# otiliastr/coper

Measured on NVIDIA B200. Metric: train_rows_per_s, higher is better.
Workload: dtype fp16x3

## Files before the change

### coper_b200/_lib.py

```python
from __future__ import annotations

import ctypes as C
import os

_HERE = os.path.dirname(os.path.abspath(__file__))
LIB_PATH = os.path.join(_HERE, "libcoper_sm100.so")

PREC = {"fp32": 0, "bf16": 1, "tf32x3": 2, "fp16x3": 3}
CPG_BWD_REUSE_FWD, CPG_BWD_INPUT_GRADS_ONLY, CPG_BWD_WEIGHT_GRADS_ONLY, CPG_BWD_DCB_ACCUMULATE = 1, 2, 4, 8

vp, i32, i64, u64, f32, sz = C.c_void_p, C.c_int, C.c_int64, C.c_uint64, C.c_float, C.c_size_t

SIGNATURES = {
    "coper_version": (i32, []),
    "coper_status_string": (C.c_char_p, [i32]),
    "coper_last_cuda_error": (i32, []),
    "coper_launch_count": (C.c_longlong, []),
    "coper_device_is_sm100": (i32, []),
    "coper_set_pdl": (i32, [i32]),
    "coper_gather_rows": (i32, [vp, i64, i64, i32, vp, i32, vp, vp]),
    "coper_gather_rows2": (i32, [vp, i64, i64, i32, vp, i32, vp, vp, i64, i64, i32, vp, i32, vp, vp, vp, f32, f32, f32, vp]),
    "coper_conv_fwd": (i32, [vp, i32, i32, i32, vp, vp, i32, i32, i32, i32, vp, vp]),
    "coper_conv_bwd_slabs": (i32, [i32, i32, i32, i32, i32, i32, i32]),
    "coper_conv_bwd": (i32, [vp, vp, i32, i32, i32, vp, i32, i32, i32, i32, vp, vp, vp, vp]),
    "coper_conv_bwd_bn": (i32, [vp, vp, vp, i32, i32, i32, vp, i32, i32, i32, i32, vp, vp, vp, vp, vp, vp, i32, f32, vp, u64,
                                vp, vp, vp, vp, vp]),
    "coper_colstats_chunks": (i32, [i64]),
    "coper_colstats": (i32, [vp, i64, i32, vp, vp]),
    "coper_bn_finalize": (i32, [vp, i32, i64, i32, vp, vp, vp, vp, f32, f32, i32, i32, i32, vp, vp, vp, vp, vp]),
    "coper_bn_stats_finalize": (i32, [vp, i64, i32, vp, vp, vp, vp, vp, vp, f32, f32, i32, i32, vp, vp, vp, vp, vp]),
    "coper_bn_act_fwd": (i32, [vp, i64, i32, vp, vp, i32, f32, vp, u64, vp, vp]),
    "coper_bn_act_fwd_moving": (i32, [vp, i64, i32, vp, vp, vp, vp, f32, i32, vp, vp]),
    "coper_bn_act_bwd_stats": (i32, [vp, vp, i64, i32, vp, vp, vp, vp, i32, f32, vp, u64, vp, vp]),
    "coper_bn_act_bwd_stats_finalize": (i32, [vp, vp, i64, i32, vp, vp, vp, vp, i32, f32, vp, u64, vp, vp, i32, vp, vp, vp, vp,
                                              vp]),
    "coper_bn_act_bwd_finalize": (i32, [vp, i32, i64, i32, i32, vp, vp, vp, vp, vp]),
    "coper_bn_act_bwd_apply": (i32, [vp, vp, i64, i32, vp, vp, vp, vp, vp, vp, i32, f32, vp, u64, f32, u64, vp, vp]),
    "coper_dropout_mask": (i32, [i64, f32, vp, u64, vp, vp]),
    "coper_dropout_apply": (i32, [vp, i64, f32, vp, u64, vp]),
    "coper_cpg_fc_fwd_workspace_bytes": (sz, [i32, i32, i32, i32, i32]),
    "coper_cpg_fc_fwd": (i32, [vp, vp, vp, vp, vp, vp, i32, i32, i32, i32, i32, f32, vp, u64, vp, vp, sz, i32, vp]),
    "coper_cpg_fc_bwd_workspace_bytes": (sz, [i32, i32, i32, i32, i32]),
    "coper_cpg_fc_bwd": (i32, [vp, vp, vp, vp, vp, vp, vp, i32, i32, i32, i32, i32, vp, vp, vp, vp, vp, vp, sz, i32, i32,
                               vp]),
    "coper_sgemm": (i32, [i32, i32, i32, i32, i32, vp, i32, vp, i32, vp, i32, i32, vp]),
    "coper_score1n_workspace_bytes": (sz, [i32, i64, i32, i32]),
    "coper_score1n_fwd": (i32, [vp, vp, vp, i32, i64, i32, vp, i64, vp, sz, i32, vp]),
    "coper_prepared_bytes": (sz, [i64, i32, i32]),
    "coper_prepare_operand": (i32, [vp, i64, i32, i64, i32, vp, vp]),
    "coper_score1n_fwd_prepared": (i32, [vp, vp, vp, i32, i64, i32, vp, i64, i32, vp]),
    "coper_tc_gemm_workspace_bytes": (sz, [i32, i32, i32, i32]),
    "coper_tc_gemm": (i32, [i32, i32, i32, i32, i32, vp, i32, vp, i32, vp, i32, i32, vp, sz, vp]),
    "coper_score1n_bce_workspace_bytes": (sz, [i32, i64, i32, i32]),
    "coper_score1n_bce_G_bytes": (sz, [i32, i64, i32]),
    "coper_score1n_bce_fwd_bwd": (i32, [vp, vp, vp, vp, vp, i32, i64, i32, f32, f32, f32, vp, vp, i64, vp, vp, vp, vp,
                                        sz, i32, vp]),
    "coper_score1n_bce_fwd_bwd_norm": (i32, [vp, vp, vp, vp, vp, i32, i64, i32, f32, f32, f32, vp, vp, i64, vp, vp, vp, vp,
                                             vp, sz, i32, vp]),
    "coper_score1n_bce_dE": (i32, [vp, i32, i64, i32, f32, vp, vp, vp, vp, sz, i32, vp]),
    "coper_sample_labels": (i32, [vp, vp, i32, i64, i32, i32, vp, u64, vp, vp, vp]),
    "coper_score_sampled_workspace_bytes": (sz, [i32, i32]),
    "coper_score_sampled_bce_fwd_bwd": (i32, [vp, vp, vp, vp, vp, i32, i32, i64, i32, f32, f32, f32, vp, vp, vp, vp, vp,
                                              vp, vp, vp, vp, sz, vp]),
    "coper_score_sampled_sharded_workspace_bytes": (sz, [i32, i32]),
    "coper_score_sampled_bce_fwd_bwd_sharded": (i32, [vp, vp, vp, vp, vp, i32, i32, i64, i32, f32, f32, f32, vp, vp, vp,
                                                      vp, vp, vp, vp, vp, i64, i64, vp, sz, vp]),
    "coper_score_candidates": (i32, [vp, vp, vp, vp, i32, i32, i32, i64, i64, vp, vp]),
    "coper_candidate_rank": (i32, [vp, vp, vp, vp, vp, i32, i32, i32, i64, i64, vp, vp, i32, vp, vp, vp]),
    "coper_csr_to_bits": (i32, [vp, vp, i32, i64, i64, vp, vp]),
    "coper_dense_to_bits": (i32, [vp, i32, i64, vp, vp]),
    "coper_gold_scores": (i32, [vp, i64, i32, i64, vp, i64, vp, vp]),
    "coper_filtered_rank": (i32, [vp, i64, i32, i64, vp, i64, vp, vp, vp, vp, vp]),
    "coper_score1n_rank_workspace_bytes": (sz, [i32, i32, i32]),
    "coper_score1n_gold_prepared": (i32, [vp, vp, vp, i32, i64, i32, vp, i64, vp, vp, sz, i32, vp]),
    "coper_score1n_rank_prepared": (i32, [vp, vp, vp, i32, i64, i32, vp, vp, vp, vp, i32, vp]),
    "coper_score1n_topk_workspace_bytes": (sz, [i32, i64, i32, i32, i32]),
    "coper_score1n_topk_prepared": (i32, [vp, vp, vp, i32, i64, i32, vp, i64, i32, vp, vp, vp, sz, i32, vp]),
    "coper_topk_scores_workspace_bytes": (sz, [i32, i64, i32]),
    "coper_topk_scores": (i32, [vp, i64, i32, i64, vp, i64, i32, vp, vp, vp, sz, vp]),
    "coper_topk_merge": (i32, [vp, vp, i32, i32, i32, vp, vp, vp]),
    "coper_csr_to_bits_t": (i32, [vp, vp, i32, i64, i64, vp, vp]),
    "coper_dense_to_bits_t": (i32, [vp, i32, i64, i64, vp, vp]),
    "coper_bits_t_set": (i32, [vp, i32, i64, i64, vp, vp]),
    "coper_segscatter_workspace_bytes": (sz, [i32]),
    "coper_segscatter_add_sq": (i32, [vp, i32, vp, i32, vp, vp, i64, i64, vp]),
    "coper_segscatter_add_norm": (i32, [vp, i32, vp, i32, vp, vp, i64, i64, vp, vp]),
    "coper_segscatter_add_pair": (i32, [vp, i32, vp, i32, vp, vp, i64, i64, vp, vp, i32, vp, i32, vp, vp, i64, i64, vp]),
    "coper_segscatter_add": (i32, [vp, i32, vp, i32, vp, i64, i64, vp, sz, vp]),
    "coper_reduce_partials": (i32, [vp, i32, i64, f32, i32, vp, vp]),
    "coper_reduce_partials2": (i32, [vp, i64, vp, vp, i64, vp, i32, f32, i32, vp]),
    "coper_sumsq": (i32, [vp, i64, i32, vp, vp]),
    "coper_clip_scale": (i32, [vp, i32, f32, vp, vp]),
    "coper_step_state_advance": (i32, [vp, vp, f32, f32, f32, vp]),
    "coper_sumsq_combine": (i32, [vp, i32, vp, i32, vp, vp]),
    "coper_mt_sumsq": (i32, [vp, i32, vp, i32, vp, vp, vp, vp]),
    "coper_clip_scale_n": (i32, [vp, i32, f32, vp, vp]),
    "coper_mt_sumsq_clip": (i32, [vp, i32, vp, i32, vp, vp, vp, i32, vp, i32, vp, i32, f32, vp, vp]),
    "coper_mt_amsgrad": (i32, [vp, vp, i32, vp, f32, f32, f32, vp, i32, vp]),
    "coper_amsgrad_step": (i32, [vp, vp, vp, vp, vp, i64, vp, f32, f32, f32, vp, i32, vp]),
}
SUMSQ_BLOCKS = 256
TOPK_MAX = 128
MT_CHUNK = 16384

_lib = None
launch_count = 0


class CoperError(RuntimeError):
    pass


def load():
    global _lib
    if _lib is not None:
        return _lib
    if not os.path.exists(LIB_PATH):
        raise CoperError(
            "libcoper_sm100.so not found at %s — build it with `python -m coper_b200.build` "
            "(there is no CPU/PyTorch fallback for the CoPER hot path)" % LIB_PATH)
    lib = C.CDLL(LIB_PATH)
    for name, (res, args) in SIGNATURES.items():
        fn = getattr(lib, name)
        fn.restype = res
        fn.argtypes = args
    _lib = lib
    return lib


def check(rc, what=""):
    if rc != 0:
        lib = load()
        msg = lib.coper_status_string(rc).decode()
        raise CoperError("%s failed: %s (status %d, cudaError %d)" % (what, msg, rc, lib.coper_last_cuda_error()))


def ptr(t):
    return None if t is None else t.data_ptr()


def stream_ptr():
    import torch
    return torch.cuda.current_stream().cuda_stream


def call_plain(name, *args):
    check(getattr(load(), name)(*args), name)


def call(name, *args):
    global launch_count
    lib = load()
    launch_count += 1
    check(getattr(lib, name)(*args, stream_ptr()), name)
```

### coper_b200/csrc/common.cuh

```cuda
#pragma once
#include <cuda_runtime.h>
#include <stdint.h>
#include "../../include/coper.h"

namespace coper {

extern thread_local int g_last_cuda_error;
extern long long g_launch_count;

inline int check_launch() {
  ++g_launch_count;
  cudaError_t e = cudaPeekAtLastError();
  if (e != cudaSuccess) {
    g_last_cuda_error = (int)e;
    cudaGetLastError();
    return COPER_ERR_CUDA;
  }
  return COPER_OK;
}
inline int check_cuda(cudaError_t e) {
  if (e != cudaSuccess) {
    g_last_cuda_error = (int)e;
    return COPER_ERR_CUDA;
  }
  return COPER_OK;
}
#define COPER_CHECK_ARG(cond) \
  do {                        \
    if (!(cond)) return COPER_ERR_INVALID_ARG; \
  } while (0)

static inline cudaStream_t as_stream(coper_stream_t s) { return reinterpret_cast<cudaStream_t>(s); }

__device__ __forceinline__ void pdl_trigger() { asm volatile("griddepcontrol.launch_dependents;" ::: "memory"); }
__device__ __forceinline__ void pdl_wait() { asm volatile("griddepcontrol.wait;" ::: "memory"); }
__device__ __forceinline__ void pdl_enter() {
  pdl_trigger();
  pdl_wait();
}
bool pdl_enabled();
template <typename... KArgs, typename... Args>
inline void launch_pdl(void (*kernel)(KArgs...), dim3 grid, dim3 block, size_t smem, cudaStream_t st, Args&&... args) {
  cudaLaunchConfig_t cfg = {};
  cfg.gridDim = grid;
  cfg.blockDim = block;
  cfg.dynamicSmemBytes = smem;
  cfg.stream = st;
  cudaLaunchAttribute attr[1];
  attr[0].id = cudaLaunchAttributeProgrammaticStreamSerialization;
  attr[0].val.programmaticStreamSerializationAllowed = pdl_enabled() ? 1 : 0;
  cfg.attrs = attr;
  cfg.numAttrs = 1;
  cudaLaunchKernelEx(&cfg, kernel, static_cast<KArgs>(args)...);
}

__host__ __device__ __forceinline__ uint32_t hash32(uint64_t seed, uint64_t idx) {
  uint64_t z = seed + (idx + 1) * 0x9E3779B97F4A7C15ull;
  z = (z ^ (z >> 30)) * 0xBF58476D1CE4E5B9ull;
  z = (z ^ (z >> 27)) * 0x94D049BB133111EBull;
  z ^= (z >> 31);
  return (uint32_t)(z >> 32);
}
__host__ __device__ __forceinline__ uint32_t keep_threshold(float keep) {
  double t = (double)keep * 4294967296.0;
  if (t >= 4294967295.0) return 0xFFFFFFFFu;
  if (t <= 0.0) return 0u;
  return (uint32_t)t;
}
__device__ __forceinline__ float drop_factor(float keep, float inv_keep, uint32_t thr, uint64_t seed, uint64_t idx) {
  if (keep >= 1.0f) return 1.0f;
  return hash32(seed, idx) < thr ? inv_keep : 0.0f;
}

__device__ __forceinline__ float bn_bwd_dx(float dout, float post_factor, float xv, float ac, float bc, float mean,
                                           float invstd, float c1, float c2, int relu) {
  float g = __fmul_rn(dout, post_factor);
  if (relu && !(fmaf(ac, xv, bc) > 0.f)) g = 0.f;
  const float xhat = __fmul_rn(__fsub_rn(xv, mean), invstd);
  return __fmul_rn(ac, fmaf(-xhat, c2, __fsub_rn(g, c1)));
}

__device__ __forceinline__ float warp_sum(float v) {
#pragma unroll
  for (int o = 16; o > 0; o >>= 1) v += __shfl_xor_sync(0xffffffffu, v, o);
  return v;
}
__device__ __forceinline__ float warp_max(float v) {
#pragma unroll
  for (int o = 16; o > 0; o >>= 1) v = fmaxf(v, __shfl_xor_sync(0xffffffffu, v, o));
  return v;
}
__device__ __forceinline__ double warp_sum_d(double v) {
#pragma unroll
  for (int o = 16; o > 0; o >>= 1) v += __shfl_xor_sync(0xffffffffu, v, o);
  return v;
}
__device__ __forceinline__ int warp_sum_i(int v) {
#pragma unroll
  for (int o = 16; o > 0; o >>= 1) v += __shfl_xor_sync(0xffffffffu, v, o);
  return v;
}

template <typename T>
__device__ __forceinline__ T block_sum(T v, T* smem32) {
  int lane = threadIdx.x & 31, w = threadIdx.x >> 5;
#pragma unroll
  for (int o = 16; o > 0; o >>= 1) v += __shfl_xor_sync(0xffffffffu, v, o);
  if (lane == 0) smem32[w] = v;
  __syncthreads();
  T r = T(0);
  if (w == 0) {
    int nw = (blockDim.x + 31) >> 5;
    r = lane < nw ? smem32[lane] : T(0);
#pragma unroll
    for (int o = 16; o > 0; o >>= 1) r += __shfl_xor_sync(0xffffffffu, r, o);
  }
  __syncthreads();
  return r;
}

constexpr int kFp16x3TargetExp = 10;
__host__ __device__ __forceinline__ int fp16x3_exponent_of(float absmax) {
  if (!(absmax > 0.f) || !(absmax < 3.0e38f)) return 0;
  int ex;
  frexpf(absmax, &ex);
  int e = kFp16x3TargetExp - (ex - 1);
  return e < -100 ? -100 : (e > 100 ? 100 : e);
}

inline int sm_count() {
  static int cached[64] = {};
  int dev = 0;
  if (cudaGetDevice(&dev) != cudaSuccess || dev < 0 || dev >= 64) return 148;
  if (!cached[dev]) {
    int n = 0;
    if (cudaDeviceGetAttribute(&n, cudaDevAttrMultiProcessorCount, dev) != cudaSuccess || n <= 0) n = 148;
    cached[dev] = n;
  }
  return cached[dev];
}

int reduce_partials_and_sum(const float* in, int S, int64_t n, float scale, int accumulate, float* out,
                            const double* dsum_in, int dsum_n, double* dsum_out, cudaStream_t st);

static inline int ceil_div(int64_t a, int64_t b) { return (int)((a + b - 1) / b); }
static inline size_t align_up(size_t x, size_t a) { return (x + a - 1) / a * a; }

}
```

### coper_b200/csrc/umma.cuh

```cuda
#pragma once
#include <cuda.h>
#include <cuda_bf16.h>
#include "common.cuh"

namespace coper {
namespace umma {

__device__ __forceinline__ uint32_t smem_u32(const void* p) { return (uint32_t)__cvta_generic_to_shared(p); }

__device__ __forceinline__ bool elect_one() {
  uint32_t pred;
  asm volatile("{\n\t.reg .pred P;\n\telect.sync _|P, 0xffffffff;\n\tselp.u32 %0, 1, 0, P;\n\t}" : "=r"(pred));
  return pred != 0;
}
__device__ __forceinline__ int warp_idx_uniform() { return __shfl_sync(0xffffffffu, (int)(threadIdx.x >> 5), 0); }

__device__ __forceinline__ void mbar_init(uint64_t* bar, uint32_t count) {
  asm volatile("mbarrier.init.shared::cta.b64 [%0], %1;" ::"r"(smem_u32(bar)), "r"(count));
}
__device__ __forceinline__ void fence_barrier_init() { asm volatile("fence.mbarrier_init.release.cluster;" ::: "memory"); }
__device__ __forceinline__ void fence_proxy_async() { asm volatile("fence.proxy.async.shared::cta;" ::: "memory"); }
__device__ __forceinline__ void mbar_expect_tx(uint64_t* bar, uint32_t bytes) {
  asm volatile("mbarrier.arrive.expect_tx.shared::cta.b64 _, [%0], %1;" ::"r"(smem_u32(bar)), "r"(bytes) : "memory");
}
__device__ __forceinline__ void mbar_arrive(uint64_t* bar) {
  asm volatile("mbarrier.arrive.shared::cta.b64 _, [%0];" ::"r"(smem_u32(bar)) : "memory");
}
__device__ __forceinline__ void mbar_wait(uint64_t* bar, uint32_t parity) {
  uint32_t addr = smem_u32(bar);
  uint32_t done = 0;
  while (!done) {
    asm volatile(
        "{\n\t.reg .pred p;\n\t"
        "mbarrier.try_wait.parity.shared::cta.b64 p, [%1], %2;\n\t"
        "selp.u32 %0, 1, 0, p;\n\t}"
        : "=r"(done)
        : "r"(addr), "r"(parity)
        : "memory");
  }
}

__device__ __forceinline__ void tma_load_2d(void* dst_smem, const CUtensorMap* tmap, uint64_t* bar, int c0, int c1) {
  asm volatile(
      "cp.async.bulk.tensor.2d.shared::cluster.global.mbarrier::complete_tx::bytes [%0], [%1, {%3, %4}], [%2];"
      ::"r"(smem_u32(dst_smem)), "l"(reinterpret_cast<uint64_t>(tmap)), "r"(smem_u32(bar)), "r"(c0), "r"(c1)
      : "memory");
}
__device__ __forceinline__ void tma_store_2d(const CUtensorMap* tmap, const void* src_smem, int c0, int c1) {
  asm volatile("cp.async.bulk.tensor.2d.global.shared::cta.bulk_group [%0, {%2, %3}], [%1];"
               ::"l"(reinterpret_cast<uint64_t>(tmap)), "r"(smem_u32(src_smem)), "r"(c0), "r"(c1)
               : "memory");
}
__device__ __forceinline__ void tma_store_commit() { asm volatile("cp.async.bulk.commit_group;" ::: "memory"); }
__device__ __forceinline__ void tma_store_wait_read() { asm volatile("cp.async.bulk.wait_group.read 0;" ::: "memory"); }
__device__ __forceinline__ void tma_store_wait_all() { asm volatile("cp.async.bulk.wait_group 0;" ::: "memory"); }
__device__ __forceinline__ void mbar_wait_guarded(uint64_t* bar, uint32_t parity) {
  uint32_t addr = smem_u32(bar);
  uint32_t done = 0;
  long long t0 = 0;
  for (uint32_t spins = 0; !done; ++spins) {
    asm volatile(
        "{\n\t.reg .pred p;\n\t"
        "mbarrier.try_wait.parity.shared::cta.b64 p, [%1], %2;\n\t"
        "selp.u32 %0, 1, 0, p;\n\t}"
        : "=r"(done)
        : "r"(addr), "r"(parity)
        : "memory");
    if (!done && (spins & 1023u) == 1023u) {
      long long now = clock64();
      if (t0 == 0) t0 = now;
      else if (now - t0 > 4000000000ll) __trap();
    }
  }
}
__device__ __forceinline__ void tma_prefetch_l2_2d(const CUtensorMap* tmap, int c0, int c1) {
  asm volatile("cp.async.bulk.prefetch.tensor.2d.L2.global.tile [%0, {%1, %2}];"
               ::"l"(reinterpret_cast<uint64_t>(tmap)), "r"(c0), "r"(c1)
               : "memory");
}
__device__ __forceinline__ void tma_prefetch_desc(const CUtensorMap* tmap) {
  asm volatile("prefetch.tensormap [%0];" ::"l"(reinterpret_cast<uint64_t>(tmap)) : "memory");
}

__device__ __forceinline__ void tmem_alloc(uint32_t* smem_dst, uint32_t ncols) {
  asm volatile("tcgen05.alloc.cta_group::1.sync.aligned.shared::cta.b32 [%0], %1;" ::"r"(smem_u32(smem_dst)), "r"(ncols)
               : "memory");
}
__device__ __forceinline__ void tmem_relinquish() {
  asm volatile("tcgen05.relinquish_alloc_permit.cta_group::1.sync.aligned;" ::: "memory");
}
__device__ __forceinline__ void tmem_dealloc(uint32_t taddr, uint32_t ncols) {
  asm volatile("tcgen05.dealloc.cta_group::1.sync.aligned.b32 %0, %1;" ::"r"(taddr), "r"(ncols) : "memory");
}
__device__ __forceinline__ void tc_fence_before() { asm volatile("tcgen05.fence::before_thread_sync;" ::: "memory"); }
__device__ __forceinline__ void tc_fence_after() { asm volatile("tcgen05.fence::after_thread_sync;" ::: "memory"); }

__device__ __forceinline__ void mma_bf16(uint32_t tmem_d, uint64_t desc_a, uint64_t desc_b, uint32_t idesc, uint32_t acc) {
  asm volatile(
      "{\n\t.reg .pred p;\n\tsetp.ne.b32 p, %4, 0;\n\t"
      "tcgen05.mma.cta_group::1.kind::f16 [%0], %1, %2, %3, p;\n\t}"
      ::"r"(tmem_d), "l"(desc_a), "l"(desc_b), "r"(idesc), "r"(acc)
      : "memory");
}
__device__ __forceinline__ void mma_tf32(uint32_t tmem_d, uint64_t desc_a, uint64_t desc_b, uint32_t idesc, uint32_t acc) {
  asm volatile(
      "{\n\t.reg .pred p;\n\tsetp.ne.b32 p, %4, 0;\n\t"
      "tcgen05.mma.cta_group::1.kind::tf32 [%0], %1, %2, %3, p;\n\t}"
      ::"r"(tmem_d), "l"(desc_a), "l"(desc_b), "r"(idesc), "r"(acc)
      : "memory");
}
__device__ __forceinline__ void mma_commit(uint64_t* bar) {
  asm volatile("tcgen05.commit.cta_group::1.mbarrier::arrive::one.shared::cluster.b64 [%0];" ::"r"(smem_u32(bar))
               : "memory");
}

__device__ __forceinline__ void tmem_ld32(uint32_t taddr, uint32_t (&r)[32]) {
  asm volatile(
      "tcgen05.ld.sync.aligned.32x32b.x32.b32 "
      "{%0, %1, %2, %3, %4, %5, %6, %7, %8, %9, %10, %11, %12, %13, %14, %15, "
      "%16, %17, %18, %19, %20, %21, %22, %23, %24, %25, %26, %27, %28, %29, %30, %31}, [%32];"
      : "=r"(r[0]), "=r"(r[1]), "=r"(r[2]), "=r"(r[3]), "=r"(r[4]), "=r"(r[5]), "=r"(r[6]), "=r"(r[7]), "=r"(r[8]),
        "=r"(r[9]), "=r"(r[10]), "=r"(r[11]), "=r"(r[12]), "=r"(r[13]), "=r"(r[14]), "=r"(r[15]), "=r"(r[16]),
        "=r"(r[17]), "=r"(r[18]), "=r"(r[19]), "=r"(r[20]), "=r"(r[21]), "=r"(r[22]), "=r"(r[23]), "=r"(r[24]),
        "=r"(r[25]), "=r"(r[26]), "=r"(r[27]), "=r"(r[28]), "=r"(r[29]), "=r"(r[30]), "=r"(r[31])
      : "r"(taddr)
      : "memory");
}
__device__ __forceinline__ void tmem_ld16(uint32_t taddr, uint32_t (&r)[16]) {
  asm volatile(
      "tcgen05.ld.sync.aligned.32x32b.x16.b32 "
      "{%0, %1, %2, %3, %4, %5, %6, %7, %8, %9, %10, %11, %12, %13, %14, %15}, [%16];"
      : "=r"(r[0]), "=r"(r[1]), "=r"(r[2]), "=r"(r[3]), "=r"(r[4]), "=r"(r[5]), "=r"(r[6]), "=r"(r[7]), "=r"(r[8]),
        "=r"(r[9]), "=r"(r[10]), "=r"(r[11]), "=r"(r[12]), "=r"(r[13]), "=r"(r[14]), "=r"(r[15])
      : "r"(taddr)
      : "memory");
}
__device__ __forceinline__ void tmem_ld_wait() { asm volatile("tcgen05.wait::ld.sync.aligned;" ::: "memory"); }

enum : uint32_t { LAYOUT_SW128 = 2, LAYOUT_SW128_BASE32B = 1 };
__device__ __forceinline__ uint64_t make_desc(uint32_t smem_addr, uint32_t lbo_bytes, uint32_t sbo_bytes,
                                              uint32_t layout_type = LAYOUT_SW128) {
  uint64_t d = 0;
  d |= (uint64_t)((smem_addr & 0x3FFFFu) >> 4);
  d |= (uint64_t)((lbo_bytes >> 4) & 0x3FFFu) << 16;
  d |= (uint64_t)((sbo_bytes >> 4) & 0x3FFFu) << 32;
  d |= (uint64_t)1 << 46;
  d |= (uint64_t)layout_type << 61;
  return d;
}
__device__ __forceinline__ uint64_t make_desc_kmajor(uint32_t smem_addr) { return make_desc(smem_addr, 16, 1024); }

enum : uint32_t { FMT_F16 = 0, FMT_BF16 = 1, FMT_TF32 = 2 };
__host__ __device__ constexpr uint32_t make_idesc(uint32_t fmt, uint32_t M, uint32_t N, uint32_t a_mn, uint32_t b_mn) {
  return (1u << 4) | (fmt << 7) | (fmt << 10) | (a_mn << 15) | (b_mn << 16) | ((N >> 3) << 17) | ((M >> 4) << 24);
}

typedef CUresult (*EncodeTiledFn)(CUtensorMap*, CUtensorMapDataType, cuuint32_t, void*, const cuuint64_t*,
                                  const cuuint64_t*, const cuuint32_t*, const cuuint32_t*, CUtensorMapInterleave,
                                  CUtensorMapSwizzle, CUtensorMapL2promotion, CUtensorMapFloatOOBfill);
EncodeTiledFn get_encode_fn();

int make_tmap_2d(CUtensorMap* out, const void* base, int elem_bytes, bool is_bf16, uint64_t rows, uint64_t cols,
                 uint64_t pitch_elems, uint32_t box_cols, uint32_t box_rows, bool atom32 = false);

}
}
```

### coper_b200/csrc/umma_cpg.cu

```cuda
#include <cuda_fp16.h>
#include "umma_gemm.cuh"

namespace coper {
using namespace umma;

size_t tc_prepared_bytes(int64_t rows, int cols, int prec);
int tc_prepare(const float* src, int64_t rows, int cols, int64_t ld_src, int prec, void* dst, cudaStream_t st);
int64_t tc_prepared_ld(int cols, int prec);
TcOperand tc_operand(const void* prep, int64_t rows, int cols, int prec);
void* tc_fp16x3_trailer(const void* prep, int64_t rows, int cols);
int tc_gemm_store(int prec, bool a_mn, bool b_mn, const TcOperand& A, const TcOperand& B, const GemmProblem& p,
                  bool split, const StoreEpi& epi, cudaStream_t st);

struct CpgFwdEpi : EpiBase {
  static constexpr bool kAccumulate = true;
  const float* c;
  int dc;
  float* out;
  long long ld, split_stride;
  __device__ __forceinline__ float group_scale(const GemmProblem& p, const TileCoord& t, int row) const {
    return row < p.M ? __ldg(c + (long long)row * dc + t.group) : 0.f;
  }
  __device__ __forceinline__ void chunk(const GemmProblem& p, const TileCoord& t, int row, int col,
                                        const uint32_t (&r)[32], int) const {
    if (row >= p.M) return;
    float* o = out + t.split * split_stride + (long long)row * ld + col;
    if (col + 31 < p.N && ((reinterpret_cast<uintptr_t>(o) & 15) == 0)) {
#pragma unroll
      for (int j = 0; j < 32; j += 4)
        *reinterpret_cast<float4*>(o + j) = make_float4(__uint_as_float(r[j]), __uint_as_float(r[j + 1]),
                                                        __uint_as_float(r[j + 2]), __uint_as_float(r[j + 3]));
    } else {
#pragma unroll
      for (int j = 0; j < 32; ++j)
        if (col + j < p.N) o[j] = __uint_as_float(r[j]);
    }
  }
};

template <int PREC>
using CpgFwdCfg = GemmCfg<PREC, 256, (PREC == PREC_BF16 ? 4 : 2), 8, false, true,
                          (PREC == PREC_BF16 ? 0 : PREC == PREC_FP16X3 ? 2 : 4)>;

struct CpgFwdPlan {
  GemmProblem p;
  size_t off_f, off_P, off_slabs, total;
};
static CpgFwdPlan cpg_fwd_plan(int B, int dc, int F, int d, int prec) {
  CpgFwdPlan L;
  GemmProblem p{};
  p.M = B; p.N = d; p.K = F; p.groups = dc; p.groups_inner = 1;
  p.a_group_mn = 0; p.a_group_k = 0; p.b_group_mn = 0; p.b_group_k = F;
  if (prec == COPER_PREC_BF16) plan_gemm<CpgFwdCfg<PREC_BF16>>(p, true);
  else if (prec == COPER_PREC_FP16X3) plan_gemm<CpgFwdCfg<PREC_FP16X3>>(p, true);
  else plan_gemm<CpgFwdCfg<PREC_TF32X3>>(p, true);
  L.p = p;
  size_t o = 0;
  L.off_f = o; o = align_up(o + tc_prepared_bytes(B, F, prec), 256);
  L.off_P = o; o = align_up(o + tc_prepared_bytes((int64_t)dc * F, d, prec), 256);
  L.off_slabs = o; o = align_up(o + (size_t)p.splits * B * d * sizeof(float), 256);
  L.total = o;
  return L;
}

struct CpgBwdTEpi : EpiBase {
  static constexpr bool kAccumulate = true;
  const float* c;
  const float* f;
  int dc;
  float* df;
  float* dc_part;
  float freg[32];
  float fsum;
  __device__ __forceinline__ void tile_begin(const GemmProblem& p, const TileCoord&, int row, int col0) {
    fsum = 0.f;
    if (row < p.M && col0 < p.N) {
      const float4* src = reinterpret_cast<const float4*>(f + (long long)row * p.N + col0);
#pragma unroll
      for (int j = 0; j < 8; ++j) {
        float4 v = __ldg(src + j);
        freg[4 * j] = v.x; freg[4 * j + 1] = v.y; freg[4 * j + 2] = v.z; freg[4 * j + 3] = v.w;
      }
    } else {
#pragma unroll
      for (int j = 0; j < 32; ++j) freg[j] = 0.f;
    }
  }
  __device__ __forceinline__ float group_scale(const GemmProblem& p, const TileCoord& t, int row) const {
    return row < p.M ? __ldg(c + (long long)row * dc + t.group) : 0.f;
  }
  __device__ __forceinline__ void group_vals(const GemmProblem&, const TileCoord&, int, int, const uint32_t (&v)[16],
                                             int half_idx) {
#pragma unroll
    for (int j = 0; j < 16; ++j) fsum = fmaf(freg[(half_idx & 1) * 16 + j], __uint_as_float(v[j]), fsum);
  }
  __device__ __forceinline__ void group_done(const GemmProblem& p, const TileCoord& t, int row, int col_group,
                                             int col_groups) {
    if (row < p.M)
      dc_part[((long long)(t.n_blk * col_groups + col_group) * p.M + row) * dc + t.group] = fsum;
    fsum = 0.f;
  }
  __device__ __forceinline__ void chunk(const GemmProblem& p, const TileCoord&, int row, int col,
                                        const uint32_t (&r)[32], int) const {
    if (row >= p.M) return;
    float4* o = reinterpret_cast<float4*>(df + (long long)row * p.N + col);
#pragma unroll
    for (int j = 0; j < 8; ++j)
      o[j] = make_float4(__uint_as_float(r[4 * j]), __uint_as_float(r[4 * j + 1]), __uint_as_float(r[4 * j + 2]),
                         __uint_as_float(r[4 * j + 3]));
  }
};
constexpr int kBwdTEpiWarps = 16;
constexpr int kBwdTBlockN = 128;
template <int PREC>
using CpgBwdTCfg = GemmCfg<PREC, kBwdTBlockN, (PREC == PREC_BF16 ? 4 : 3), kBwdTEpiWarps, false, false, 0>;

__global__ void absmax_scaled_kernel(const float* __restrict__ dy, const float* __restrict__ c, int B, int d, int dc,
                                     uint32_t* __restrict__ trailer) {
  pdl_enter();
  const int lane = threadIdx.x & 31;
  for (int b = blockIdx.x * (blockDim.x >> 5) + (threadIdx.x >> 5); b < B; b += gridDim.x * (blockDim.x >> 5)) {
    float my = 0.f, mc = 0.f;
    for (int j = lane; j < d; j += 32) my = fmaxf(my, fabsf(__ldg(dy + (int64_t)b * d + j)));
    for (int g = lane; g < dc; g += 32) mc = fmaxf(mc, fabsf(__ldg(c + (int64_t)b * dc + g)));
#pragma unroll
    for (int o = 16; o > 0; o >>= 1) {
      my = fmaxf(my, __shfl_xor_sync(0xffffffffu, my, o));
      mc = fmaxf(mc, __shfl_xor_sync(0xffffffffu, mc, o));
    }
    const float m = my * mc;
    if (lane == 0 && m > 0.f) atomicMax(trailer + 1, __float_as_uint(m));
  }
}
__global__ void prepare_scaled_kernel(const float* __restrict__ dy, const float* __restrict__ c, int B, int d, int dc,
                                      int64_t ldp, int prec, void* __restrict__ dst, uint32_t* __restrict__ trailer) {
  pdl_enter();
  int64_t n = (int64_t)dc * B * ldp;
  int64_t stride = (int64_t)gridDim.x * blockDim.x;
  float sc = 1.0f;
  if (prec == COPER_PREC_FP16X3) {
    const int ex = fp16x3_exponent_of(__uint_as_float(trailer[1]));
    if (blockIdx.x == 0 && threadIdx.x == 0) reinterpret_cast<int*>(trailer)[0] = ex;
    sc = exp2f((float)ex);
  }
  for (int64_t e = (int64_t)blockIdx.x * blockDim.x + threadIdx.x; e < n; e += stride) {
    int64_t r = e / ldp;
    int j = (int)(e - r * ldp);
    int g = (int)(r / B), b = (int)(r - (int64_t)g * B);
    float x = j < d ? __ldg(dy + (int64_t)b * d + j) * __ldg(c + (int64_t)b * dc + g) : 0.f;
    if (prec == COPER_PREC_BF16) {
      static_cast<__nv_bfloat16*>(dst)[e] = __float2bfloat16_rn(x);
    } else if (prec == COPER_PREC_FP16X3) {
      const float xs = x * sc;
      const __half h = __float2half_rn(xs);
      static_cast<__half*>(dst)[e] = h;
      static_cast<__half*>(dst)[n + e] = __float2half_rn(xs - __half2float(h));
    } else {
      uint32_t h;
      asm("cvt.rna.tf32.f32 %0, %1;" : "=r"(h) : "f"(x));
      float hf = __uint_as_float(h);
      static_cast<float*>(dst)[e] = hf;
      static_cast<float*>(dst)[n + e] = x - hf;
    }
  }
}

__global__ void __launch_bounds__(256) cpg_bwd_prepare_fp16x3_kernel(const float* __restrict__ dy,
                                                                     const float* __restrict__ c, int B, int d, int dc,
                                                                     int64_t ldp, __half* __restrict__ dyp,
                                                                     __half* __restrict__ dycp,
                                                                     uint32_t* __restrict__ tr_dy,
                                                                     uint32_t* __restrict__ tr_dyc) {
  pdl_enter();
  __shared__ float wmax[2][8];
  const int lane = threadIdx.x & 31, warp = threadIdx.x >> 5;
  float m_dy = 0.f, m_dyc = 0.f;
  for (int b = blockIdx.x * 8 + warp; b < B; b += gridDim.x * 8) {
    float my = 0.f, mc = 0.f;
    for (int j = lane; j < d; j += 32) my = fmaxf(my, fabsf(__ldg(dy + (int64_t)b * d + j)));
    for (int g = lane; g < dc; g += 32) mc = fmaxf(mc, fabsf(__ldg(c + (int64_t)b * dc + g)));
    my = warp_max(my);
    mc = warp_max(mc);
    m_dy = fmaxf(m_dy, my);
    m_dyc = fmaxf(m_dyc, my * mc);
  }
  if (lane == 0) { wmax[0][warp] = m_dy; wmax[1][warp] = m_dyc; }
  __syncthreads();
  if (threadIdx.x == 0) {
#pragma unroll
    for (int w = 1; w < 8; ++w) { m_dy = fmaxf(m_dy, wmax[0][w]); m_dyc = fmaxf(m_dyc, wmax[1][w]); }
    if (m_dy > 0.f) atomicMax(tr_dy + 1, __float_as_uint(m_dy));
    if (m_dyc > 0.f) atomicMax(tr_dy + 4, __float_as_uint(m_dyc));
    __threadfence();
    atomicAdd(tr_dy + 3, 1u);
    const long long t0 = clock64();
    while (*reinterpret_cast<volatile uint32_t*>(tr_dy + 3) < gridDim.x) {
      if (clock64() - t0 > 4000000000ll) __trap();
    }
    __threadfence();
  }
  __syncthreads();
  const uint32_t bits_dy = *reinterpret_cast<volatile uint32_t*>(tr_dy + 1);
  const uint32_t bits_dyc = *reinterpret_cast<volatile uint32_t*>(tr_dy + 4);
  const int e_dy = fp16x3_exponent_of(__uint_as_float(bits_dy)), e_dyc = fp16x3_exponent_of(__uint_as_float(bits_dyc));
  if (blockIdx.x == 0 && threadIdx.x == 0) {
    reinterpret_cast<int*>(tr_dy)[0] = e_dy;
    tr_dy[2] = bits_dy;
    reinterpret_cast<int*>(tr_dyc)[0] = e_dyc;
    tr_dyc[1] = bits_dyc;
  }
  const float sc_dy = exp2f((float)e_dy), sc_dyc = exp2f((float)e_dyc);
  const int gpr = (int)(ldp / 8);
  const int64_t per = (int64_t)B * gpr, units = per * (1 + dc);
  __half* const dy_lo = dyp + (int64_t)B * ldp;
  __half* const dyc_lo = dycp + (int64_t)dc * B * ldp;
  for (int64_t u = (int64_t)blockIdx.x * 256 + threadIdx.x; u < units; u += (int64_t)gridDim.x * 256) {
    const int p = (int)(u / per);
    const int64_t v = u - (int64_t)p * per;
    const int b = (int)(v / gpr), c0 = (int)(v - (int64_t)b * gpr) * 8;
    const float cs = p == 0 ? 1.0f : __ldg(c + (int64_t)b * dc + (p - 1));
    const float sc = p == 0 ? sc_dy : sc_dyc;
    __half2 h[4], l[4];
#pragma unroll
    for (int k = 0; k < 4; ++k) {
      const int j = c0 + 2 * k;
      float x0 = j < d ? __ldg(dy + (int64_t)b * d + j) : 0.f, x1 = j + 1 < d ? __ldg(dy + (int64_t)b * d + j + 1) : 0.f;
      if (p != 0) { x0 = j < d ? x0 * cs : 0.f; x1 = j + 1 < d ? x1 * cs : 0.f; }
      const float a0 = x0 * sc, a1 = x1 * sc;
      h[k] = __floats2half2_rn(a0, a1);
      const float2 hf = __half22float2(h[k]);
      l[k] = __floats2half2_rn(a0 - hf.x, a1 - hf.y);
    }
    __half* hi = p == 0 ? dyp + v * 8 : dycp + ((int64_t)(p - 1) * per + v) * 8;
    __half* lo = p == 0 ? dy_lo + v * 8 : dyc_lo + ((int64_t)(p - 1) * per + v) * 8;
    *reinterpret_cast<uint4*>(hi) = *reinterpret_cast<uint4*>(h);
    *reinterpret_cast<uint4*>(lo) = *reinterpret_cast<uint4*>(l);
  }
}

struct CpgBwdPlan {
  size_t off_f, off_P, off_dy, off_dyc, off_dcpart, total;
  int dc_slabs;
};
static CpgBwdPlan cpg_bwd_plan(int B, int dc, int F, int d, int prec) {
  CpgBwdPlan L;
  size_t o = 0;
  L.off_f = o; o = align_up(o + tc_prepared_bytes(B, F, prec), 256);
  L.off_P = o; o = align_up(o + tc_prepared_bytes((int64_t)dc * F, d, prec), 256);
  L.off_dy = o; o = align_up(o + tc_prepared_bytes(B, d, prec), 256);
  L.off_dyc = o; o = align_up(o + tc_prepared_bytes((int64_t)dc * B, d, prec), 256);
  L.dc_slabs = ((F + kBwdTBlockN - 1) / kBwdTBlockN) * (kBwdTEpiWarps / 4);
  L.off_dcpart = o; o = align_up(o + (size_t)L.dc_slabs * B * dc * sizeof(float), 256);
  L.total = o;
  return L;
}

size_t umma_cpg_fwd_workspace_bytes(int B, int dc, int F, int d, int prec) { return cpg_fwd_plan(B, dc, F, d, prec).total; }
size_t umma_cpg_bwd_workspace_bytes(int B, int dc, int F, int d, int prec) {
  size_t a = cpg_bwd_plan(B, dc, F, d, prec).total, b = cpg_fwd_plan(B, dc, F, d, prec).total;
  return a > b ? a : b;
}

int umma_cpg_fwd_partials(const float* c, const float* f, const float* P, const void* P_prepared, int B, int dc, int F,
                          int d, void* ws, size_t ws_bytes, int prec, cudaStream_t st, float** slabs, int* n_slabs) {
  if (F % 32 != 0 || d > 256) return COPER_ERR_UNSUPPORTED;
  CpgFwdPlan L = cpg_fwd_plan(B, dc, F, d, prec);
  if (!ws || ws_bytes < L.total) return COPER_ERR_WORKSPACE;
  if (reinterpret_cast<uintptr_t>(ws) & 255) return COPER_ERR_INVALID_ARG;
  char* w = static_cast<char*>(ws);
  void* fp = w + L.off_f;
  const void* Pp = P_prepared ? P_prepared : w + L.off_P;
  float* out = reinterpret_cast<float*>(w + L.off_slabs);
  int rc;
  if ((rc = tc_prepare(f, B, F, F, prec, fp, st))) return rc;
  if (!P_prepared && (rc = tc_prepare(P, (int64_t)dc * F, d, d, prec, w + L.off_P, st))) return rc;
  CpgFwdEpi epi;
  epi.c = c; epi.dc = dc; epi.out = out; epi.ld = d; epi.split_stride = (long long)B * d;
  TcOperand A = tc_operand(fp, B, F, prec), Bo = tc_operand(Pp, (int64_t)dc * F, d, prec);
  if (prec == COPER_PREC_BF16) rc = launch_gemm<CpgFwdCfg<PREC_BF16>, CpgFwdEpi>(A, Bo, L.p, epi, st);
  else if (prec == COPER_PREC_FP16X3) rc = launch_gemm<CpgFwdCfg<PREC_FP16X3>, CpgFwdEpi>(A, Bo, L.p, epi, st);
  else rc = launch_gemm<CpgFwdCfg<PREC_TF32X3>, CpgFwdEpi>(A, Bo, L.p, epi, st);
  *slabs = out;
  *n_slabs = L.p.splits;
  return rc;
}

int umma_cpg_bwd(const float* c, const float* f, const float* P, const void* P_prepared, const float* dy, int B, int dc,
                 int F, int d, float* dP, float* df, float* dc_out, void* ws, size_t ws_bytes, int prec,
                 int flags, cudaStream_t st) {
  if (F % 32 != 0 || d > 256) return COPER_ERR_UNSUPPORTED;
  const bool inputs = !(flags & COPER_CPG_BWD_WEIGHT_GRADS_ONLY), weights = !(flags & COPER_CPG_BWD_INPUT_GRADS_ONLY);
  CpgBwdPlan L = cpg_bwd_plan(B, dc, F, d, prec);
  if (!ws || ws_bytes < L.total) return COPER_ERR_WORKSPACE;
  if (reinterpret_cast<uintptr_t>(ws) & 255) return COPER_ERR_INVALID_ARG;
  char* w = static_cast<char*>(ws);
  void* fp = w + L.off_f;
  const void* Pp = P_prepared ? P_prepared : w + L.off_P;
  void* dyp = w + L.off_dy;
  void* dycp = w + L.off_dyc;
  float* dc_part = reinterpret_cast<float*>(w + L.off_dcpart);
  int rc = COPER_OK;
  if (inputs) {
    if (!(flags & COPER_CPG_BWD_REUSE_FWD)) {
      if ((rc = tc_prepare(f, B, F, F, prec, fp, st))) return rc;
      if (!P_prepared && (rc = tc_prepare(P, (int64_t)dc * F, d, d, prec, w + L.off_P, st))) return rc;
    }
    int64_t ldp = tc_prepared_ld(d, prec);
    int64_t n = (int64_t)dc * B * ldp;
    if (prec == COPER_PREC_FP16X3 && n <= ((int64_t)8 << 20)) {
      uint32_t* tr_dy = static_cast<uint32_t*>(tc_fp16x3_trailer(dyp, B, d));
      uint32_t* tr_dyc = static_cast<uint32_t*>(tc_fp16x3_trailer(dycp, (int64_t)dc * B, d));
      if ((rc = check_cuda(cudaMemsetAsync(tr_dy, 0, 32, st)))) return rc;
      const int64_t want = ((int64_t)(1 + dc) * B * (ldp / 8) + 256 * 4 - 1) / (256 * 4);
      int g = (int)(want < (int64_t)sm_count() * 2 ? want : (int64_t)sm_count() * 2);
      if (g < 1) g = 1;
      launch_pdl(cpg_bwd_prepare_fp16x3_kernel, g, 256, 0, st, dy, c, B, d, dc, ldp, static_cast<__half*>(dyp),
                 static_cast<__half*>(dycp), tr_dy, tr_dyc);
      if ((rc = check_launch())) return rc;
    } else {
      if ((rc = tc_prepare(dy, B, d, d, prec, dyp, st))) return rc;
      int grid = (int)((n + 255) / 256 < sm_count() * 8 ? (n + 255) / 256 : sm_count() * 8);
      uint32_t* trailer = nullptr;
      if (prec == COPER_PREC_FP16X3) {
        trailer = static_cast<uint32_t*>(tc_fp16x3_trailer(dycp, (int64_t)dc * B, d));
        if ((rc = check_cuda(cudaMemsetAsync(trailer, 0, 8, st)))) return rc;
        launch_pdl(absmax_scaled_kernel, (B + 7) / 8, 256, 0, st, dy, c, B, d, dc, trailer);
        if ((rc = check_launch())) return rc;
      }
      launch_pdl(prepare_scaled_kernel, grid, 256, 0, st, dy, c, B, d, dc, ldp, prec, dycp, trailer);
      if ((rc = check_launch())) return rc;
    }
    GemmProblem p{};
    p.M = B; p.N = F; p.K = d; p.groups = dc; p.groups_inner = 1;
    p.a_group_mn = 0; p.a_group_k = 0; p.b_group_mn = F; p.b_group_k = 0;
    CpgBwdTEpi epi;
    epi.c = c; epi.f = f; epi.dc = dc; epi.df = df; epi.dc_part = dc_part; epi.fsum = 0.f;
    TcOperand A = tc_operand(dyp, B, d, prec), Bo = tc_operand(Pp, (int64_t)dc * F, d, prec);
    if (prec == COPER_PREC_BF16) {
      plan_gemm<CpgBwdTCfg<PREC_BF16>>(p, false);
      rc = launch_gemm<CpgBwdTCfg<PREC_BF16>, CpgBwdTEpi>(A, Bo, p, epi, st);
    } else if (prec == COPER_PREC_FP16X3) {
      plan_gemm<CpgBwdTCfg<PREC_FP16X3>>(p, false);
      rc = launch_gemm<CpgBwdTCfg<PREC_FP16X3>, CpgBwdTEpi>(A, Bo, p, epi, st);
    } else {
      plan_gemm<CpgBwdTCfg<PREC_TF32X3>>(p, false);
      rc = launch_gemm<CpgBwdTCfg<PREC_TF32X3>, CpgBwdTEpi>(A, Bo, p, epi, st);
    }
    if (rc) return rc;
    if ((rc = coper_reduce_partials(dc_part, L.dc_slabs, (int64_t)B * dc, 1.0f, 0, dc_out, (coper_stream_t)st)))
      return rc;
  }
  if (weights) {
    GemmProblem p{};
    p.M = F; p.N = d; p.K = B; p.groups = dc; p.groups_inner = 0;
    p.a_group_mn = 0; p.a_group_k = 0; p.b_group_mn = 0; p.b_group_k = B;
    StoreEpi epi = make_store_epi(dP, d, (long long)F * d, 0);
    rc = tc_gemm_store(prec, true, true, tc_operand(fp, B, F, prec), tc_operand(dycp, (int64_t)dc * B, d, prec), p,
                       false, epi, st);
  }
  return rc;
}

}
```

### coper_b200/csrc/umma_entity.cu

```cuda
#include <cuda_fp16.h>
#include "umma_gemm.cuh"
#include "bce_math.cuh"

namespace coper {
using namespace umma;

size_t tc_prepared_bytes(int64_t rows, int cols, int prec);
int tc_prepare(const float* src, int64_t rows, int cols, int64_t ld_src, int prec, void* dst, cudaStream_t st);
int64_t tc_prepared_ld(int cols, int prec);
TcOperand tc_operand(const void* prep, int64_t rows, int cols, int prec);
void* tc_fp16x3_trailer(const void* prep, int64_t rows, int cols);
int tc_gemm_store(int prec, bool a_mn, bool b_mn, const TcOperand& A, const TcOperand& B, const GemmProblem& p,
                  bool split, const StoreEpi& epi, cudaStream_t st);
int tc_plan_splits(int prec, GemmProblem p, bool split);
bool umma_fused_ok(int B, int64_t Ns, int d, int prec);
void umma_fused_plan(int B, int64_t Ns, int* QB, int* R);
int umma_bce_dq_fused(const TcOperand& E, const TcOperand& Q, const float* bias, const uint32_t* bitsT, int B, int64_t Ns,
                      int d, float pos, float neg, float inv_count, void* GT, int64_t ldGT, float* dq_part,
                      float* dbias_part, double* loss_part, int* grid_out, cudaStream_t st);

constexpr int kEntEpiWarps = 16;
constexpr int kBceEpiWarps = 16;

template <int NCH>
struct RowState {
  const float* bias;
  const uint32_t* bitsT;
  int wordsB;
  float bias_cur, bias_nx;
  uint32_t w_cur[NCH], w_nx[NCH];
  int nx_row, nx_col0;
  __device__ __forceinline__ void load(const GemmProblem& p, int row, int col0, float& b, uint32_t (&w)[NCH]) const {
    const int rc = min(row, p.M - 1);
    b = __ldg(bias + rc);
#pragma unroll
    for (int i = 0; i < NCH; ++i) {
      const int col = min(col0 + i * 32, ((p.N - 1) >> 5) << 5);
      w[i] = bitsT ? __ldg(bitsT + (int64_t)rc * wordsB + (col >> 5)) : 0u;
    }
  }
  __device__ __forceinline__ void begin(const GemmProblem& p, int row, int col0) {
    if (nx_row == row && nx_col0 == col0) {
      bias_cur = bias_nx;
#pragma unroll
      for (int i = 0; i < NCH; ++i) w_cur[i] = w_nx[i];
    } else {
      load(p, row, col0, bias_cur, w_cur);
    }
  }
  __device__ __forceinline__ void prefetch(const GemmProblem& p, int row, int col0) {
    load(p, row, col0, bias_nx, w_nx);
    nx_row = row;
    nx_col0 = col0;
  }
  __host__ void init(const float* bias_, const uint32_t* bitsT_, int wordsB_) {
    bias = bias_; bitsT = bitsT_; wordsB = wordsB_;
    bias_cur = bias_nx = 0.f;
    nx_row = nx_col0 = -1;
    for (int i = 0; i < NCH; ++i) w_cur[i] = w_nx[i] = 0;
  }
};

template <int NCH>
struct ScoreEpiT : EpiBase {
  RowState<NCH> rs;
  float* out;
  int64_t ld;
  __device__ __forceinline__ void tile_begin(const GemmProblem& p, const TileCoord&, int row, int col0) { rs.begin(p, row, col0); }
  __device__ __forceinline__ void tile_prefetch(const GemmProblem& p, const TileCoord&, int row, int col0) { rs.prefetch(p, row, col0); }
  __device__ __forceinline__ void chunk(const GemmProblem& p, const TileCoord&, int row, int col, const uint32_t (&r)[32],
                                        int) const {
    if (row >= p.M) return;
    float* o = out + (int64_t)col * ld + row;
#pragma unroll
    for (int j = 0; j < 32; ++j)
      if (col + j < p.N) o[(int64_t)j * ld] = __uint_as_float(r[j]) + rs.bias_cur;
  }
};

template <int PREC, int NCH>
struct BceEpiT : EpiBase {
  RowState<NCH> rs;
  float pos, neg, inv_count;
  float rsum_scale;
  void* GT;
  int64_t ldGT;
  float* dbias_part;
  double* loss_part;
  double loss_acc;
  float rsum;
  __device__ __forceinline__ void tile_begin(const GemmProblem& p, const TileCoord&, int row, int col0) {
    rs.begin(p, row, col0);
    rsum = 0.f;
  }
  __device__ __forceinline__ void tile_prefetch(const GemmProblem& p, const TileCoord&, int row, int col0) { rs.prefetch(p, row, col0); }

  template <bool GENERAL>
  __device__ __forceinline__ void body(const uint32_t (&r)[32], uint32_t w, uint32_t vm, float (&g)[32], float& lsum,
                                       float& gsum) const {
    if (GENERAL) {
      bce_chunk_general(r, rs.bias_cur, w, vm, pos, neg, inv_count, g, lsum, gsum);
    } else {
      bce_chunk_dense(r, rs.bias_cur, neg, inv_count, g, lsum, gsum);
    }
  }
  __device__ __forceinline__ void chunk(const GemmProblem& p, const TileCoord&, int row, int col, const uint32_t (&r)[32],
                                        int ci) {
    const bool rowok = row < p.M;
    const int ncol = p.N - col;
    const uint32_t vm = ncol >= 32 ? 0xFFFFFFFFu : ((1u << ncol) - 1u);
    const uint32_t w = rowok ? (rs.w_cur[ci] & vm) : 0u;
    float g[32];
    float lsum, gsum;
    if (ncol < 32 || __any_sync(0xffffffffu, w != 0u)) body<true>(r, w, vm, g, lsum, gsum);
    else body<false>(r, w, vm, g, lsum, gsum);
    uint4 pk[4];
    uint4 pk2[4];
    if (rowok) {
      loss_acc += (double)lsum;
      rsum += gsum * rsum_scale;
      if (PREC == PREC_FP16X3) {
#pragma unroll
        for (int v = 0; v < 4; ++v) {
          uint32_t hw[4], lw[4];
#pragma unroll
          for (int k = 0; k < 4; ++k) {
            const float a = g[8 * v + 2 * k], b = g[8 * v + 2 * k + 1];
            const __half2 h = __floats2half2_rn(a, b);
            const float2 hf = __half22float2(h);
            const __half2 l = __floats2half2_rn(a - hf.x, b - hf.y);
            hw[k] = *reinterpret_cast<const uint32_t*>(&h);
            lw[k] = *reinterpret_cast<const uint32_t*>(&l);
          }
          pk[v] = make_uint4(hw[0], hw[1], hw[2], hw[3]);
          pk2[v] = make_uint4(lw[0], lw[1], lw[2], lw[3]);
        }
      } else if (PREC == PREC_BF16) {
#pragma unroll
        for (int v = 0; v < 4; ++v) {
          __nv_bfloat162 t0 = __floats2bfloat162_rn(g[8 * v], g[8 * v + 1]);
          __nv_bfloat162 t1 = __floats2bfloat162_rn(g[8 * v + 2], g[8 * v + 3]);
          __nv_bfloat162 t2 = __floats2bfloat162_rn(g[8 * v + 4], g[8 * v + 5]);
          __nv_bfloat162 t3 = __floats2bfloat162_rn(g[8 * v + 6], g[8 * v + 7]);
          pk[v].x = *reinterpret_cast<uint32_t*>(&t0); pk[v].y = *reinterpret_cast<uint32_t*>(&t1);
          pk[v].z = *reinterpret_cast<uint32_t*>(&t2); pk[v].w = *reinterpret_cast<uint32_t*>(&t3);
        }
      } else if (PREC == PREC_TF32X3) {
        float* hi = static_cast<float*>(GT) + (int64_t)col * ldGT + row;
        float* lo = hi + (int64_t)p.N * ldGT;
#pragma unroll
        for (int j = 0; j < 32; ++j) {
          if (j < ncol) {
            uint32_t hb;
            asm("cvt.rna.tf32.f32 %0, %1;" : "=r"(hb) : "f"(g[j]));
            *hi = __uint_as_float(hb);
            *lo = g[j] - __uint_as_float(hb);
          }
          hi += ldGT;
          lo += ldGT;
        }
      }
    }
    if (PREC == PREC_BF16 || PREC == PREC_FP16X3) {
      __shared__ uint4 stage_g[kBceEpiWarps][128];
      uint4* st = stage_g[(threadIdx.x >> 5) - 4];
      const int lane = threadIdx.x & 31;
      const int row0 = row - lane;
      const int64_t ld16 = ldGT / 8;
      const int gq = lane & 3;
#pragma unroll
      for (int plane = 0; plane < (PREC == PREC_FP16X3 ? 2 : 1); ++plane) {
#pragma unroll
        for (int v = 0; v < 4; ++v) st[lane * 4 + (v ^ ((lane >> 1) & 3))] = plane ? pk2[v] : pk[v];
        __syncwarp();
        uint4* o0 = reinterpret_cast<uint4*>(static_cast<uint16_t*>(GT) + ((int64_t)plane * p.M + row0) * ldGT + col);
#pragma unroll
        for (int k = 0; k < 4; ++k) {
          const int rr = 8 * k + (lane >> 2);
          const uint4 x = st[rr * 4 + (gq ^ ((rr >> 1) & 3))];
          if (row0 + rr < p.M) o0[(int64_t)rr * ld16 + gq] = x;
        }
        __syncwarp();
      }
    }
  }
  __device__ __forceinline__ void tile_done(const GemmProblem& p, const TileCoord& t, int row, int col_group, int col_groups) {
    if (row < p.M) dbias_part[(int64_t)(t.n_blk * col_groups + col_group) * p.M + row] = rsum;
  }
  __device__ __forceinline__ void finish(int epi_thread, int epi_threads) {
    double t = warp_sum_d(loss_acc);
    if ((epi_thread & 31) == 0) loss_part[(int64_t)blockIdx.x * (epi_threads >> 5) + (epi_thread >> 5)] = t;
  }
};

constexpr int kRankPlanes = 8;
template <int NCH>
struct RankEpiT : EpiBase {
  RowState<NCH> rs;
  const float* gold;
  int32_t* n_greater;
  int32_t* n_equal;
  uint32_t planes[NCH][kRankPlanes];
  int ce[NCH];
  int cur_col0, n_queries, adds;
  __device__ __forceinline__ float* gold_smem() {
    __shared__ float gold_s[kEntEpiWarps][NCH * 32];
    return gold_s[(threadIdx.x >> 5) - 4];
  }
  __device__ __forceinline__ void flush() {
    const int lane = threadIdx.x & 31;
    if (cur_col0 >= 0) {
#pragma unroll
      for (int i = 0; i < NCH; ++i) {
        int v[32];
#pragma unroll
        for (int j = 0; j < 32; ++j) {
          int c = 0;
#pragma unroll
          for (int k = 0; k < kRankPlanes; ++k) c |= (int)((planes[i][k] >> j) & 1u) << k;
          v[j] = c;
        }
#pragma unroll
        for (int k = 0; k < kRankPlanes; ++k) planes[i][k] = 0;
#pragma unroll
        for (int off = 16; off >= 1; off >>= 1) {
          const bool upper = (lane & off) != 0;
#pragma unroll
          for (int q = 0; q < off; ++q) {
            const int send = upper ? v[q] : v[q + off];
            const int keepv = upper ? v[q + off] : v[q];
            v[q] = keepv + __shfl_xor_sync(0xffffffffu, send, off);
          }
        }
        const int cnt = v[0];
        const int col = cur_col0 + i * 32 + lane;
        if (col < n_queries) {
          if (cnt) atomicAdd(n_greater + col, cnt);
          if (ce[i]) atomicAdd(n_equal + col, ce[i]);
        }
        ce[i] = 0;
      }
    }
    adds = 0;
  }
  __device__ __forceinline__ void tile_begin(const GemmProblem& p, const TileCoord&, int row, int col0) {
    if (col0 != cur_col0 || adds >= (1 << kRankPlanes) - 1) {
      const bool reload = col0 != cur_col0;
      flush();
      cur_col0 = col0;
      if (reload) {
        float* gs = gold_smem();
        const int lane = threadIdx.x & 31;
        __syncwarp();
#pragma unroll
        for (int k = 0; k < NCH; ++k) {
          const int c = col0 + k * 32 + lane;
          gs[k * 32 + lane] = c < p.N ? __ldg(gold + c) : 0.f;
        }
        __syncwarp();
      }
    }
    rs.begin(p, row, col0);
  }
  __device__ __forceinline__ void tile_prefetch(const GemmProblem& p, const TileCoord&, int row, int col0) { rs.prefetch(p, row, col0); }
  __device__ __forceinline__ void chunk(const GemmProblem& p, const TileCoord&, int row, int, const uint32_t (&r)[32], int ci) {
    const float* gs = gold_smem() + ci * 32;
    uint32_t mgr = 0, mner = 0;
#pragma unroll
    for (int j = 0; j < 32; ++j) {
      const float s = __uint_as_float(r[j]) + rs.bias_cur;
      const float x = gs[j] - s;
      float ne;
      asm("add.rn.f32 %0, %1, 0f00000000;" : "=f"(ne) : "f"(-fabsf(x)));
      mgr = __funnelshift_l(__float_as_uint(x), mgr, 1);
      mner = __funnelshift_l(__float_as_uint(ne), mner, 1);
    }
    uint32_t mg = __brev(mgr), me = ~__brev(mner);
    uint32_t keep = ~rs.w_cur[ci];
    if (row >= p.M) keep = 0u;
    mg &= keep;
    me &= keep;
    uint32_t carry = mg;
#pragma unroll
    for (int k = 0; k < kRankPlanes; ++k) {
      const uint32_t t = planes[ci][k] & carry;
      planes[ci][k] ^= carry;
      carry = t;
    }
    if (__any_sync(0xffffffffu, me != 0)) {
      const int lane = threadIdx.x & 31;
#pragma unroll 1
      for (int j = 0; j < 32; ++j) {
        const uint32_t be = __ballot_sync(0xffffffffu, (me >> j) & 1u);
        if (lane == j) ce[ci] += __popc(be);
      }
    }
  }
  __device__ __forceinline__ void tile_done(const GemmProblem&, const TileCoord&, int, int, int) { ++adds; }
  __device__ __forceinline__ void finish(int, int) { flush(); }
};

struct DiagEpiT : EpiBase {
  const float* bias;
  const int64_t* e2;
  int64_t ent_lo, Ns;
  float* gold;
  __device__ __forceinline__ void chunk(const GemmProblem& p, const TileCoord&, int row, int col, const uint32_t (&r)[32],
                                        int) const {
    if (row >= p.M || row < col || row >= col + 32) return;
    int64_t l = e2[row] - ent_lo;
    float v = 0.f;
    if (l >= 0 && l < Ns) {
      float acc = 0.f;
#pragma unroll
      for (int j = 0; j < 32; ++j) acc = (col + j == row) ? __uint_as_float(r[j]) : acc;
      v = acc + __ldg(bias + l);
    }
    gold[row] = v;
  }
};

__device__ __noinline__ void topk_heap_push(uint64_t* h, int k, uint64_t key) {
  if (key <= h[0]) return;
  int i = 0;
  for (;;) {
    const int l = 2 * i + 1;
    if (l >= k) break;
    uint64_t hc = h[l];
    int c = l;
    if (l + 1 < k) {
      const uint64_t hr = h[l + 1];
      if (hr < hc) { hc = hr; c = l + 1; }
    }
    if (hc >= key) break;
    h[i] = hc;
    i = c;
  }
  h[i] = key;
}
__device__ __forceinline__ float topk_key_score(uint64_t key) {
  if (key == 0ull) return -INFINITY;
  const uint32_t u = (uint32_t)(key >> 32);
  if (u == 0x80000000u) return -0.f;
  return __uint_as_float((u & 0x80000000u) ? (u & 0x7FFFFFFFu) : ~u);
}
template <int NCH>
struct TopkEpiT : EpiBase {
  RowState<NCH> rs;
  uint64_t* lists;
  int k, cur_col0;
  uint32_t id_hi;
  __device__ __forceinline__ float* tau_smem() {
    __shared__ float tau_s[kEntEpiWarps][NCH * 32];
    return tau_s[(threadIdx.x >> 5) - 4];
  }
  __device__ __forceinline__ uint64_t* heap(const GemmProblem& p, int col) const {
    return lists + ((int64_t)(blockIdx.x * 4 + ((threadIdx.x >> 5) & 3)) * p.N + col) * k;
  }
  __device__ __forceinline__ void tile_begin(const GemmProblem& p, const TileCoord&, int row, int col0) {
    if (col0 != cur_col0) {
      cur_col0 = col0;
      float* ts = tau_smem();
      const int lane = threadIdx.x & 31;
      __syncwarp();
#pragma unroll
      for (int i = 0; i < NCH; ++i) {
        const int c = col0 + i * 32 + lane;
        ts[i * 32 + lane] = c < p.N ? topk_key_score(heap(p, c)[0]) : INFINITY;
      }
      __syncwarp();
    }
    rs.begin(p, row, col0);
  }
  __device__ __forceinline__ void tile_prefetch(const GemmProblem& p, const TileCoord&, int row, int col0) { rs.prefetch(p, row, col0); }
  __device__ __forceinline__ void chunk(const GemmProblem& p, const TileCoord&, int row, int col, const uint32_t (&r)[32],
                                        int ci) {
    float* ts = tau_smem() + ci * 32;
    uint32_t msk = 0;
#pragma unroll
    for (int j = 0; j < 32; ++j) {
      const float x = (__uint_as_float(r[j]) + rs.bias_cur) - ts[j];
      msk = __funnelshift_l(__float_as_uint(x), msk, 1);
    }
    uint32_t cand = ~__brev(msk) & ~rs.w_cur[ci];
    if (row >= p.M) cand = 0u;
    if (p.N - col < 32) cand &= (1u << (p.N - col)) - 1u;
    if (!__any_sync(0xffffffffu, cand != 0u)) return;
    const int lane = threadIdx.x & 31;
    const uint32_t cols = __reduce_or_sync(0xffffffffu, cand);
    const uint32_t key_lo0 = id_hi - (uint32_t)(row - lane);
#pragma unroll
    for (int j = 0; j < 32; ++j) {
      if ((cols >> j) & 1u) {
        uint32_t rows = __ballot_sync(0xffffffffu, (cand >> j) & 1u);
        const float sj = __uint_as_float(r[j]) + rs.bias_cur;
        uint64_t* h = heap(p, col + j);
        while (rows) {
          const int src = __ffs(rows) - 1;
          rows &= rows - 1;
          const float v = __shfl_sync(0xffffffffu, sj, src);
          if (lane == j) {
            uint32_t u = __float_as_uint(v == 0.f ? 0.f : v);
            u = (u & 0x80000000u) ? ~u : (u | 0x80000000u);
            const uint32_t lo = ((key_lo0 - (uint32_t)src) << 1) | (uint32_t)(__float_as_uint(v) == 0x80000000u);
            topk_heap_push(h, k, ((uint64_t)u << 32) | (uint64_t)lo);
          }
        }
        if (lane == j) ts[j] = topk_key_score(h[0]);
      }
    }
    __syncwarp();
  }
};

__global__ void gather_prepared_kernel(const uint4* __restrict__ src, int64_t Ns, int vec_per_row, int planes,
                                       const int64_t* __restrict__ e2, int64_t ent_lo, int B, uint4* __restrict__ dst,
                                       const int* __restrict__ src_exp, int* __restrict__ dst_exp) {
  pdl_enter();
  int b = blockIdx.x;
  if (src_exp && b == 0 && threadIdx.x == 0) *dst_exp = *src_exp;
  int64_t l = e2[b] - ent_lo;
  bool owned = l >= 0 && l < Ns;
  for (int pl = 0; pl < planes; ++pl) {
    const uint4* s = src + ((int64_t)pl * Ns + (owned ? l : 0)) * vec_per_row;
    uint4* o = dst + ((int64_t)pl * B + b) * vec_per_row;
    for (int v = threadIdx.x; v < vec_per_row; v += blockDim.x) o[v] = owned ? __ldg(s + v) : make_uint4(0, 0, 0, 0);
  }
}

__global__ void sum_doubles_kernel(const double* __restrict__ in, int n, double* out) {
  pdl_enter();
  __shared__ double smd[32];
  double acc = 0.0;
  for (int i = threadIdx.x; i < n; i += blockDim.x) acc += in[i];
  double t = block_sum<double>(acc, smd);
  if (threadIdx.x == 0) *out = t;
}

template <int PREC, bool RES>
struct EntSel;
template <>
struct EntSel<PREC_BF16, true> { using Cfg = GemmCfg<PREC_BF16, 256, 5, kEntEpiWarps, false, false, 0, 4>; };
template <>
struct EntSel<PREC_BF16, false> { using Cfg = GemmCfg<PREC_BF16, 128, 6, kEntEpiWarps, false, false, 0, 0>; };
template <>
struct EntSel<PREC_TF32X3, false> { using Cfg = GemmCfg<PREC_TF32X3, 128, 3, kEntEpiWarps, false, false, 0, 0>; };
template <>
struct EntSel<PREC_FP16X3, false> { using Cfg = GemmCfg<PREC_FP16X3, 128, 3, kEntEpiWarps, false, false, 0, 0>; };
template <>
struct EntSel<PREC_FP16X3, true> { using Cfg = GemmCfg<PREC_FP16X3, 128, 2, kEntEpiWarps, false, false, 0, 4>; };
template <int PREC, bool RES>
struct BceSel;
template <>
struct BceSel<PREC_BF16, true> { using Cfg = GemmCfg<PREC_BF16, 256, 3, kBceEpiWarps, false, false, 0, 4>; };
template <>
struct BceSel<PREC_BF16, false> { using Cfg = GemmCfg<PREC_BF16, 128, 5, kBceEpiWarps, false, false, 0, 0>; };
template <>
struct BceSel<PREC_TF32X3, false> { using Cfg = GemmCfg<PREC_TF32X3, 128, 3, kBceEpiWarps, false, false, 0, 0>; };
template <>
struct BceSel<PREC_FP16X3, false> { using Cfg = GemmCfg<PREC_FP16X3, 128, 3, kBceEpiWarps, false, false, 0, 0>; };
template <>
struct BceSel<PREC_FP16X3, true> { using Cfg = GemmCfg<PREC_FP16X3, 128, 2, kBceEpiWarps, false, false, 0, 4>; };
template <class Cfg>
constexpr int ent_nch() { return Cfg::BLOCK_N / (Cfg::EPI_WARPS / 4) / 32; }
static inline bool ent_resident(int d, int prec, int64_t Ns, int B) {
  if ((prec != COPER_PREC_BF16 && prec != COPER_PREC_FP16X3) || d > 256) return false;
  const int bn = prec == COPER_PREC_BF16 ? 256 : 128;
  const int64_t tiles = ((Ns + BLOCK_M - 1) / BLOCK_M) * ((B + bn - 1) / bn);
  return tiles >= 8 * (int64_t)sm_count();
}
static inline int ent_block_n(int d, int prec, int64_t Ns, int B) {
  return (prec == COPER_PREC_BF16 && ent_resident(d, prec, Ns, B)) ? 256 : 128;
}

static GemmProblem ent_problem(int B, int64_t Ns, int d, int block_n) {
  GemmProblem p{};
  p.M = (int)Ns; p.N = B; p.K = d; p.groups = 1; p.groups_inner = 0;
  p.m_tiles = (int)((Ns + BLOCK_M - 1) / BLOCK_M);
  p.n_tiles = (B + block_n - 1) / block_n;
  p.splits = 1;
  p.kb_per_split = 1 << 28;
  p.n_fastest = 1;
  return p;
}
static int ent_grid(const GemmProblem& p) {
  long long supers = (long long)p.m_tiles * p.n_tiles;
  const int sms = sm_count();
  int grid = (int)(supers < sms ? supers : sms);
  if (p.n_tiles <= grid) grid = grid / p.n_tiles * p.n_tiles;
  return grid;
}

template <class Cfg>
static int score_t_impl(const TcOperand& E, const TcOperand& Q, const float* bias, int B, int64_t Ns, int d, float* S,
                        int64_t ld, cudaStream_t st) {
  GemmProblem p = ent_problem(B, Ns, d, Cfg::BLOCK_N);
  ScoreEpiT<ent_nch<Cfg>()> epi;
  epi.rs.init(bias, nullptr, 0);
  epi.out = S; epi.ld = ld;
  return launch_gemm<Cfg, ScoreEpiT<ent_nch<Cfg>()>>(E, Q, p, epi, st, ent_grid(p));
}
#define ENT_DISPATCH(FN, ...)                                                                              \
  do {                                                                                                     \
    if (prec == COPER_PREC_BF16 && ent_resident(d, prec, Ns, B)) return FN<EntSel<PREC_BF16, true>::Cfg>(__VA_ARGS__);  \
    if (prec == COPER_PREC_BF16) return FN<EntSel<PREC_BF16, false>::Cfg>(__VA_ARGS__);                   \
    if (prec == COPER_PREC_TF32X3) return FN<EntSel<PREC_TF32X3, false>::Cfg>(__VA_ARGS__);               \
    if (prec == COPER_PREC_FP16X3 && ent_resident(d, prec, Ns, B)) return FN<EntSel<PREC_FP16X3, true>::Cfg>(__VA_ARGS__); \
    if (prec == COPER_PREC_FP16X3) return FN<EntSel<PREC_FP16X3, false>::Cfg>(__VA_ARGS__);               \
    return COPER_ERR_UNSUPPORTED;                                                                          \
  } while (0)
int umma_score1n_fwd_prepared(const void* q_prep, const void* E_prep, const float* bias, int B, int64_t Ns, int d,
                              float* scores, int64_t ld, int prec, cudaStream_t st) {
  if (ld < Ns || Ns > 0x7fffffff - 512) return COPER_ERR_INVALID_ARG;
  TcOperand Q = tc_operand(q_prep, B, d, prec), E = tc_operand(E_prep, Ns, d, prec);
  ENT_DISPATCH(score_t_impl, E, Q, bias, B, Ns, d, scores, ld, st);
}

size_t umma_rank_workspace_bytes(int B, int d, int prec) { return align_up(tc_prepared_bytes(B, d, prec), 256); }

template <class Cfg>
static int gold_impl(const TcOperand& Eg, const TcOperand& Q, const float* bias, int B, int64_t Ns, int d,
                     const int64_t* e2, int64_t ent_lo, float* gold, cudaStream_t st) {
  GemmProblem p = ent_problem(B, B, d, Cfg::BLOCK_N);
  DiagEpiT epi;
  epi.bias = bias; epi.e2 = e2; epi.ent_lo = ent_lo; epi.Ns = Ns; epi.gold = gold;
  return launch_gemm<Cfg, DiagEpiT>(Eg, Q, p, epi, st);
}
int umma_score1n_gold(const void* q_prep, const void* E_prep, const float* bias, int B, int64_t Ns, int d,
                      const int64_t* e2, int64_t ent_lo, float* gold, void* ws, size_t ws_bytes, int prec,
                      cudaStream_t st) {
  if (!ws || ws_bytes < umma_rank_workspace_bytes(B, d, prec) || (reinterpret_cast<uintptr_t>(ws) & 255))
    return COPER_ERR_WORKSPACE;
  int64_t ldp = tc_prepared_ld(d, prec);
  int elem = prec == COPER_PREC_TF32X3 ? 4 : 2;
  int vec_per_row = (int)(ldp * elem / 16);
  const int* src_exp = nullptr;
  int* dst_exp = nullptr;
  if (prec == COPER_PREC_FP16X3) {
    src_exp = static_cast<const int*>(tc_fp16x3_trailer(E_prep, Ns, d));
    dst_exp = static_cast<int*>(tc_fp16x3_trailer(ws, B, d));
  }
  launch_pdl(gather_prepared_kernel, B, 64, 0, st, static_cast<const uint4*>(E_prep), Ns, vec_per_row, prec ==
             COPER_PREC_BF16 ? 1 : 2, e2, ent_lo, B, static_cast<uint4*>(ws), src_exp, dst_exp);
  int rc = check_launch();
  if (rc) return rc;
  TcOperand Q = tc_operand(q_prep, B, d, prec), Eg = tc_operand(ws, B, d, prec);
  ENT_DISPATCH(gold_impl, Eg, Q, bias, B, Ns, d, e2, ent_lo, gold, st);
}

template <class Cfg>
static int rank_impl(const TcOperand& E, const TcOperand& Q, const float* bias, int B, int64_t Ns, int d,
                     const float* gold, const uint32_t* filtT, int32_t* n_greater, int32_t* n_equal, cudaStream_t st) {
  GemmProblem p = ent_problem(B, Ns, d, Cfg::BLOCK_N);
  constexpr int kEntNCH = ent_nch<Cfg>();
  RankEpiT<kEntNCH> epi;
  epi.rs.init(bias, filtT, (B + 31) / 32);
  epi.gold = gold; epi.n_greater = n_greater; epi.n_equal = n_equal;
  epi.cur_col0 = -1;
  epi.n_queries = B;
  epi.adds = 0;
  for (int i = 0; i < kEntNCH; ++i) {
    epi.ce[i] = 0;
    for (int k = 0; k < kRankPlanes; ++k) epi.planes[i][k] = 0;
  }
  return launch_gemm<Cfg, RankEpiT<kEntNCH>>(E, Q, p, epi, st, ent_grid(p));
}
int umma_score1n_rank(const void* q_prep, const void* E_prep, const float* bias, int B, int64_t Ns, int d,
                      const float* gold, const uint32_t* filtT, int32_t* n_greater, int32_t* n_equal, int prec,
                      cudaStream_t st) {
  if (Ns > 0x7fffffff - 512) return COPER_ERR_UNSUPPORTED;
  TcOperand Q = tc_operand(q_prep, B, d, prec), E = tc_operand(E_prep, Ns, d, prec);
  ENT_DISPATCH(rank_impl, E, Q, bias, B, Ns, d, gold, filtT, n_greater, n_equal, st);
}

int topk_merge_keys(const uint64_t* lists, int B, int k, int per, int first_div, int step, int n_groups, float* out_s,
                    int64_t* out_id, cudaStream_t st);
size_t umma_topk_workspace_bytes(int B, int k) { return align_up((size_t)sm_count() * 4 * B * k * sizeof(uint64_t), 256); }

template <class Cfg>
static int topk_impl(const TcOperand& E, const TcOperand& Q, const float* bias, int B, int64_t Ns, int d,
                     const uint32_t* filtT, int64_t ent_lo, int k, float* out_s, int64_t* out_id, void* ws,
                     cudaStream_t st) {
  GemmProblem p = ent_problem(B, Ns, d, Cfg::BLOCK_N);
  constexpr int kEntNCH = ent_nch<Cfg>();
  const int grid = ent_grid(p);
  uint64_t* lists = static_cast<uint64_t*>(ws);
  int rc = check_cuda(cudaMemsetAsync(lists, 0, (size_t)grid * 4 * B * k * sizeof(uint64_t), st));
  if (rc) return rc;
  TopkEpiT<kEntNCH> epi;
  epi.rs.init(bias, filtT, (B + 31) / 32);
  epi.lists = lists; epi.k = k; epi.cur_col0 = -1;
  epi.id_hi = 0x7FFFFFFFu - (uint32_t)ent_lo;
  if ((rc = launch_gemm<Cfg, TopkEpiT<kEntNCH>>(E, Q, p, epi, st, grid))) return rc;
  if (p.n_tiles <= grid) return topk_merge_keys(lists, B, k, 4, Cfg::BLOCK_N, p.n_tiles, grid / p.n_tiles, out_s, out_id, st);
  return topk_merge_keys(lists, B, k, 4, 0, 1, grid, out_s, out_id, st);
}
int umma_score1n_topk(const void* q_prep, const void* E_prep, const float* bias, int B, int64_t Ns, int d,
                      const uint32_t* filtT, int64_t ent_lo, int k, float* out_s, int64_t* out_id, void* ws,
                      size_t ws_bytes, int prec, cudaStream_t st) {
  if (prec != COPER_PREC_BF16 && prec != COPER_PREC_TF32X3 && prec != COPER_PREC_FP16X3) return COPER_ERR_UNSUPPORTED;
  if (Ns > 0x7fffffff - 512 || ent_lo + Ns >= 0x7FFFFFFFll) return COPER_ERR_UNSUPPORTED;
  if (!ws || ws_bytes < umma_topk_workspace_bytes(B, k) || (reinterpret_cast<uintptr_t>(ws) & 255))
    return COPER_ERR_WORKSPACE;
  TcOperand Q = tc_operand(q_prep, B, d, prec), E = tc_operand(E_prep, Ns, d, prec);
  ENT_DISPATCH(topk_impl, E, Q, bias, B, Ns, d, filtT, ent_lo, k, out_s, out_id, ws, st);
}

static int dE_gemm(int prec, bool a_mn, const TcOperand& Go, const TcOperand& Qo, const GemmProblem& p, StoreEpi epi,
                   double* dE_sumsq, double* ss_part, cudaStream_t st) {
  int rc;
  const int n_part = sm_count() * 16;
  if (dE_sumsq) {
    if ((rc = check_cuda(cudaMemsetAsync(ss_part, 0, (size_t)n_part * sizeof(double), st)))) return rc;
    epi.sumsq_part = ss_part;
  }
  if ((rc = tc_gemm_store(prec, a_mn, true, Go, Qo, p, false, epi, st))) return rc;
  if (dE_sumsq) {
    launch_pdl(sum_doubles_kernel, 1, 256, 0, st, ss_part, n_part, dE_sumsq);
    rc = check_launch();
  }
  return rc;
}
struct BceTcLayout {
  size_t off_q, off_E, off_dq, off_dbias, off_loss, off_ss, total;
  int splits, dbias_slabs;
};
static BceTcLayout bce_tc_layout(int B, int64_t Ns, int d, int prec) {
  BceTcLayout L;
  GemmProblem p{};
  p.M = B; p.N = d; p.K = (int)Ns; p.groups = 1;
  L.splits = tc_plan_splits(prec, p, true);
  int bn = ent_block_n(d, prec, Ns, B);
  L.dbias_slabs = ((B + bn - 1) / bn) * (kBceEpiWarps / 4);
  size_t dq_rows = (size_t)L.splits * B;
  if (umma_fused_ok(B, Ns, d, prec)) {
    int QB, R;
    umma_fused_plan(B, Ns, &QB, &R);
    if ((size_t)R * B > dq_rows) dq_rows = (size_t)R * B;
    if (QB > L.dbias_slabs) L.dbias_slabs = QB;
  }
  size_t o = 0;
  L.off_q = o; o = align_up(o + tc_prepared_bytes(B, d, prec), 256);
  L.off_E = o; o = align_up(o + tc_prepared_bytes(Ns, d, prec), 256);
  L.off_dq = o; o = align_up(o + dq_rows * d * sizeof(float), 256);
  L.off_dbias = o; o = align_up(o + (size_t)L.dbias_slabs * Ns * sizeof(float), 256);
  L.off_loss = o; o = align_up(o + (size_t)sm_count() * kBceEpiWarps * sizeof(double), 256);
  L.off_ss = o; o = align_up(o + (size_t)sm_count() * 16 * sizeof(double), 256);
  L.total = o;
  return L;
}
size_t umma_bce_workspace_bytes(int B, int64_t Ns, int d, int prec) { return bce_tc_layout(B, Ns, d, prec).total; }
static int bce_dbias_slabs_used(const BceTcLayout& L, int B, int64_t Ns, int d, int prec) {
  if (umma_fused_ok(B, Ns, d, prec)) {
    int QB, R;
    umma_fused_plan(B, Ns, &QB, &R);
    return QB;
  }
  int bn = ent_block_n(d, prec, Ns, B);
  (void)L;
  return ((B + bn - 1) / bn) * (kBceEpiWarps / 4);
}
static inline int64_t gt_pitch(int B) { return (B + 31) / 32 * 32; }
size_t umma_bce_G_bytes(int B, int64_t Ns, int prec) {
  if (prec == COPER_PREC_BF16) return (size_t)Ns * gt_pitch(B) * 2;
  if (prec == COPER_PREC_FP16X3) return (size_t)Ns * gt_pitch(B) * 2 * 2;
  return (size_t)B * ((Ns + 31) / 32 * 32) * 8;
}

template <class Cfg>
static int bce_impl(const TcOperand& E, const TcOperand& Q, const float* bias, const uint32_t* bitsT, int B, int64_t Ns,
                    int d, float pos, float neg, float inv_count, void* GT, int64_t ldGT, float* dbias_part,
                    double* loss_part, cudaStream_t st, int* grid_out) {
  GemmProblem p = ent_problem(B, Ns, d, Cfg::BLOCK_N);
  constexpr int kEntNCH = ent_nch<Cfg>();
  constexpr int PREC = Cfg::PREC;
  BceEpiT<PREC, kEntNCH> epi;
  epi.rs.init(bias, bitsT, (B + 31) / 32);
  epi.pos = pos; epi.neg = neg; epi.GT = GT; epi.ldGT = ldGT;
  epi.inv_count = PREC == PREC_FP16X3 ? 1024.0f : inv_count;
  epi.rsum_scale = PREC == PREC_FP16X3 ? inv_count * (1.0f / 1024.0f) : 1.0f;
  epi.dbias_part = dbias_part; epi.loss_part = loss_part; epi.loss_acc = 0.0; epi.rsum = 0.f;
  *grid_out = ent_grid(p);
  return launch_gemm<Cfg, BceEpiT<PREC, kEntNCH>>(E, Q, p, epi, st, *grid_out);
}

static TcOperand g_operand(const void* G, int B, int64_t Ns, int prec) {
  const bool entity_major = prec != COPER_PREC_TF32X3;
  const int64_t ldGT = entity_major ? gt_pitch(B) : (Ns + 31) / 32 * 32;
  TcOperand Go;
  Go.main = G;
  Go.pitch = (uint64_t)ldGT;
  Go.exp = nullptr;
  if (entity_major) {
    Go.lo = prec == COPER_PREC_FP16X3 ? static_cast<const void*>(static_cast<const uint16_t*>(G) + Ns * ldGT) : nullptr;
    Go.rows = (uint64_t)Ns; Go.cols = (uint64_t)B;
  } else {
    Go.lo = static_cast<const void*>(static_cast<const float*>(G) + (int64_t)B * ldGT);
    Go.rows = (uint64_t)B; Go.cols = (uint64_t)Ns;
  }
  return Go;
}

int umma_score1n_dE(const void* G, int B, int64_t Ns, int d, float inv_count, float* dE, double* dE_sumsq, float* dbias,
                    void* ws, size_t ws_bytes, int prec, cudaStream_t st) {
  BceTcLayout L = bce_tc_layout(B, Ns, d, prec);
  if (!ws || ws_bytes < L.total) return COPER_ERR_WORKSPACE;
  char* w = static_cast<char*>(ws);
  if (dbias) {
    int rc = coper_reduce_partials(reinterpret_cast<const float*>(w + L.off_dbias), bce_dbias_slabs_used(L, B, Ns, d, prec),
                                   Ns, 1.0f, 0, dbias, (coper_stream_t)st);
    if (rc) return rc;
  }
  TcOperand Qo = tc_operand(w + L.off_q, B, d, prec), Go = g_operand(G, B, Ns, prec);
  GemmProblem p{};
  p.M = (int)Ns; p.N = d; p.K = B; p.groups = 1; p.groups_inner = 0;
  p.post_scale = prec == COPER_PREC_FP16X3 ? inv_count * (1.0f / 1024.0f) : 0.f;
  StoreEpi epi = make_store_epi(dE, d, 0, 0);
  return dE_gemm(prec, prec == COPER_PREC_TF32X3, Go, Qo, p, epi, dE_sumsq, reinterpret_cast<double*>(w + L.off_ss), st);
}

int umma_score1n_bce_fwd_bwd(const float* q, const float* E, const void* E_prepared, const float* bias,
                             const uint32_t* label_bits_t, int B, int64_t Ns, int d, float pos, float neg,
                             float inv_count, double* loss_sum, void* G, int64_t ldG, float* dq, float* dE,
                             float* dbias, void* ws, size_t ws_bytes, int prec, double* dE_sumsq, cudaStream_t st) {
  if (Ns > 0x7fffffff - 512) return COPER_ERR_UNSUPPORTED;
  (void)ldG;
  if (reinterpret_cast<uintptr_t>(G) & 127) return COPER_ERR_INVALID_ARG;
  const bool entity_major = prec != COPER_PREC_TF32X3;
  const int64_t ldGT = entity_major ? gt_pitch(B) : (Ns + 31) / 32 * 32;
  const float g_post = prec == COPER_PREC_FP16X3 ? inv_count * (1.0f / 1024.0f) : 0.f;
  BceTcLayout L = bce_tc_layout(B, Ns, d, prec);
  if (!ws || ws_bytes < L.total) return COPER_ERR_WORKSPACE;
  if (reinterpret_cast<uintptr_t>(ws) & 255) return COPER_ERR_INVALID_ARG;
  char* w = static_cast<char*>(ws);
  void* qp = w + L.off_q;
  const void* Ep = E_prepared ? E_prepared : w + L.off_E;
  float* dq_part = reinterpret_cast<float*>(w + L.off_dq);
  float* dbias_part = reinterpret_cast<float*>(w + L.off_dbias);
  double* loss_part = reinterpret_cast<double*>(w + L.off_loss);
  int rc;
  if ((rc = tc_prepare(q, B, d, d, prec, qp, st))) return rc;
  if (!E_prepared && (rc = tc_prepare(E, Ns, d, d, prec, w + L.off_E, st))) return rc;
  TcOperand Qo = tc_operand(qp, B, d, prec), Eo = tc_operand(Ep, Ns, d, prec);
  if (umma_fused_ok(B, Ns, d, prec)) {
    int QB, R, grid = 0;
    umma_fused_plan(B, Ns, &QB, &R);
    if ((rc = umma_bce_dq_fused(Eo, Qo, bias, label_bits_t, B, Ns, d, pos, neg, inv_count, G, ldGT, dq_part, dbias_part,
                                loss_part, &grid, st)))
      return rc;
    if ((rc = reduce_partials_and_sum(dq_part, R, (int64_t)B * d, 1.0f, 0, dq, loss_part, grid * kBceEpiWarps, loss_sum, st)))
      return rc;
    if (!dE) return COPER_OK;
    return umma_score1n_dE(G, B, Ns, d, inv_count, dE, dE_sumsq, dbias, ws, ws_bytes, prec, st);
  }
  int grid = 0;
  auto run_bce = [&]() -> int {
    if (prec == COPER_PREC_BF16 && ent_resident(d, prec, Ns, B))
      return bce_impl<BceSel<PREC_BF16, true>::Cfg>(Eo, Qo, bias, label_bits_t, B, Ns, d, pos, neg, inv_count, G, ldGT,
                                                    dbias_part, loss_part, st, &grid);
    if (prec == COPER_PREC_BF16)
      return bce_impl<BceSel<PREC_BF16, false>::Cfg>(Eo, Qo, bias, label_bits_t, B, Ns, d, pos, neg, inv_count, G, ldGT,
                                                     dbias_part, loss_part, st, &grid);
    if (prec == COPER_PREC_FP16X3 && ent_resident(d, prec, Ns, B))
      return bce_impl<BceSel<PREC_FP16X3, true>::Cfg>(Eo, Qo, bias, label_bits_t, B, Ns, d, pos, neg, inv_count, G, ldGT,
                                                      dbias_part, loss_part, st, &grid);
    if (prec == COPER_PREC_FP16X3)
      return bce_impl<BceSel<PREC_FP16X3, false>::Cfg>(Eo, Qo, bias, label_bits_t, B, Ns, d, pos, neg, inv_count, G, ldGT,
                                                       dbias_part, loss_part, st, &grid);
    return bce_impl<BceSel<PREC_TF32X3, false>::Cfg>(Eo, Qo, bias, label_bits_t, B, Ns, d, pos, neg, inv_count, G, ldGT,
                                                     dbias_part, loss_part, st, &grid);
  };
  if ((rc = run_bce())) return rc;
  TcOperand Go = g_operand(G, B, Ns, prec);
  {
    GemmProblem p{};
    p.M = B; p.N = d; p.K = (int)Ns; p.groups = 1; p.groups_inner = 0;
    p.post_scale = g_post;
    StoreEpi epi = make_store_epi(dq_part, d, 0, (long long)B * d);
    if ((rc = tc_gemm_store(prec, entity_major, true, Go, Eo, p, true, epi, st))) return rc;
    if ((rc = reduce_partials_and_sum(dq_part, L.splits, (int64_t)B * d, 1.0f, 0, dq, loss_part, grid * kBceEpiWarps,
                                      loss_sum, st)))
      return rc;
  }
  if (!dE) return COPER_OK;
  return umma_score1n_dE(G, B, Ns, d, inv_count, dE, dE_sumsq, dbias, ws, ws_bytes, prec, st);
}

}

using namespace coper;

extern "C" {

size_t coper_score1n_rank_workspace_bytes(int B, int d, int prec) {
  if (prec != COPER_PREC_BF16 && prec != COPER_PREC_TF32X3 && prec != COPER_PREC_FP16X3) return 0;
  return umma_rank_workspace_bytes(B, d, prec);
}
int coper_score1n_gold_prepared(const void* q_prep, const void* E_prep, const float* bias, int B, int64_t Ns, int d,
                                const int64_t* e2, int64_t ent_lo, float* gold, void* workspace,
                                size_t workspace_bytes, int prec, coper_stream_t stream) {
  COPER_CHECK_ARG(q_prep && E_prep && bias && e2 && gold && B > 0 && Ns > 0 && d > 0);
  return umma_score1n_gold(q_prep, E_prep, bias, B, Ns, d, e2, ent_lo, gold, workspace, workspace_bytes, prec,
                           as_stream(stream));
}
int coper_score1n_rank_prepared(const void* q_prep, const void* E_prep, const float* bias, int B, int64_t Ns, int d,
                                const float* gold, const uint32_t* filter_bits_t, int32_t* n_greater,
                                int32_t* n_equal, int prec, coper_stream_t stream) {
  COPER_CHECK_ARG(q_prep && E_prep && bias && gold && filter_bits_t && n_greater && n_equal);
  COPER_CHECK_ARG(B > 0 && Ns > 0 && d > 0);
  return umma_score1n_rank(q_prep, E_prep, bias, B, Ns, d, gold, filter_bits_t, n_greater, n_equal, prec,
                           as_stream(stream));
}

size_t coper_score1n_topk_workspace_bytes(int B, int64_t Ns, int d, int k, int prec) {
  if (prec != COPER_PREC_BF16 && prec != COPER_PREC_TF32X3 && prec != COPER_PREC_FP16X3) return 0;
  if (B <= 0 || Ns <= 0 || d <= 0 || k < 1 || k > COPER_TOPK_MAX) return 0;
  return umma_topk_workspace_bytes(B, k);
}
int coper_score1n_topk_prepared(const void* q_prep, const void* E_prep, const float* bias, int B, int64_t Ns, int d,
                                const uint32_t* filter_bits_t, int64_t ent_lo, int k, float* out_scores,
                                int64_t* out_ids, void* workspace, size_t workspace_bytes, int prec,
                                coper_stream_t stream) {
  COPER_CHECK_ARG(q_prep && E_prep && bias && out_scores && out_ids && B > 0 && Ns > 0 && d > 0 && ent_lo >= 0);
  COPER_CHECK_ARG(k >= 1 && k <= COPER_TOPK_MAX);
  return umma_score1n_topk(q_prep, E_prep, bias, B, Ns, d, filter_bits_t, ent_lo, k, out_scores, out_ids, workspace,
                           workspace_bytes, prec, as_stream(stream));
}

}
```

### coper_b200/csrc/umma_gemm.cu

```cuda
#include "umma_gemm.cuh"

namespace coper {
using namespace umma;

size_t tc_prepared_bytes(int64_t rows, int cols, int prec);
int tc_prepare(const float* src, int64_t rows, int cols, int64_t ld_src, int prec, void* dst, cudaStream_t st);
int64_t tc_prepared_ld(int cols, int prec);
void* tc_fp16x3_trailer(const void* prep, int64_t rows, int cols);

template <int PREC, bool A_MN, bool B_MN>
using StoreCfg = GemmCfg<PREC, 256, (PREC == PREC_BF16 ? 4 : 2), (PREC == PREC_BF16 ? 4 : 8), A_MN, B_MN,
                         (PREC == PREC_BF16 ? 0 : PREC == PREC_FP16X3 ? 2 : 4)>;

template <int PREC>
static int dispatch_layout(bool a_mn, bool b_mn, const TcOperand& A, const TcOperand& B, GemmProblem p, bool split,
                           const StoreEpi& epi, cudaStream_t st) {
  if (!a_mn && !b_mn) { plan_gemm<StoreCfg<PREC, false, false>>(p, split); return launch_gemm<StoreCfg<PREC, false, false>>(A, B, p, epi, st); }
  if (!a_mn && b_mn)  { plan_gemm<StoreCfg<PREC, false, true>>(p, split);  return launch_gemm<StoreCfg<PREC, false, true>>(A, B, p, epi, st); }
  if (a_mn && !b_mn)  { plan_gemm<StoreCfg<PREC, true, false>>(p, split);  return launch_gemm<StoreCfg<PREC, true, false>>(A, B, p, epi, st); }
  plan_gemm<StoreCfg<PREC, true, true>>(p, split);
  return launch_gemm<StoreCfg<PREC, true, true>>(A, B, p, epi, st);
}

using ResBCfg = GemmCfg<PREC_BF16, 128, 4, 8, false, true, 0, 8>;
int tc_gemm_store_resident_b(const TcOperand& A, const TcOperand& B, GemmProblem p, const StoreEpi& epi, cudaStream_t st) {
  plan_gemm<ResBCfg>(p, false);
  return launch_gemm<ResBCfg>(A, B, p, epi, st);
}
bool tc_resident_b_ok(int prec, bool a_mn, bool b_mn, const GemmProblem& p) {
  return prec == COPER_PREC_BF16 && !a_mn && b_mn && p.groups == 1 && p.K <= ResBCfg::RES_KB * ResBCfg::BLOCK_K &&
         p.M >= 16 * BLOCK_M;
}

int tc_gemm_store(int prec, bool a_mn, bool b_mn, const TcOperand& A, const TcOperand& B, const GemmProblem& p,
                  bool split, const StoreEpi& epi, cudaStream_t st) {
  if (prec == COPER_PREC_BF16) return dispatch_layout<PREC_BF16>(a_mn, b_mn, A, B, p, split, epi, st);
  if (prec == COPER_PREC_TF32X3) return dispatch_layout<PREC_TF32X3>(a_mn, b_mn, A, B, p, split, epi, st);
  if (prec == COPER_PREC_FP16X3) return dispatch_layout<PREC_FP16X3>(a_mn, b_mn, A, B, p, split, epi, st);
  return COPER_ERR_UNSUPPORTED;
}
int tc_plan_splits(int prec, GemmProblem p, bool split) {
  if (prec == COPER_PREC_BF16) plan_gemm<StoreCfg<PREC_BF16, false, false>>(p, split);
  else if (prec == COPER_PREC_FP16X3) plan_gemm<StoreCfg<PREC_FP16X3, false, false>>(p, split);
  else plan_gemm<StoreCfg<PREC_TF32X3, false, false>>(p, split);
  return p.splits;
}

TcOperand tc_operand(const void* prep, int64_t rows, int cols, int prec) {
  TcOperand o;
  int64_t ldp = tc_prepared_ld(cols, prec);
  o.main = prep;
  o.lo = prec == COPER_PREC_TF32X3 ? static_cast<const void*>(static_cast<const float*>(prep) + rows * ldp)
         : prec == COPER_PREC_FP16X3 ? static_cast<const void*>(static_cast<const uint16_t*>(prep) + rows * ldp)
                                     : nullptr;
  o.exp = prec == COPER_PREC_FP16X3 ? static_cast<const int*>(tc_fp16x3_trailer(prep, rows, cols)) : nullptr;
  o.rows = (uint64_t)rows;
  o.cols = (uint64_t)cols;
  o.pitch = (uint64_t)ldp;
  return o;
}
}

using namespace coper;

extern "C" {

size_t coper_tc_gemm_workspace_bytes(int M, int N, int K, int prec) {
  size_t a = tc_prepared_bytes(M > K ? M : K, M > K ? K : M, prec) + tc_prepared_bytes(K, M, prec);
  size_t b = tc_prepared_bytes(N > K ? N : K, N > K ? K : N, prec) + tc_prepared_bytes(K, N, prec);
  return a + b + 1024;
}

int coper_tc_gemm(int transA, int transB, int M, int N, int K, const float* A, int lda, const float* B, int ldb,
                  float* C, int ldc, int prec, void* workspace, size_t workspace_bytes, coper_stream_t stream) {
  COPER_CHECK_ARG(A && B && C && workspace && M > 0 && N > 0 && K > 0 && ldc >= N);
  if (prec != COPER_PREC_BF16 && prec != COPER_PREC_TF32X3 && prec != COPER_PREC_FP16X3) return COPER_ERR_UNSUPPORTED;
  if (workspace_bytes < coper_tc_gemm_workspace_bytes(M, N, K, prec)) return COPER_ERR_WORKSPACE;
  cudaStream_t st = as_stream(stream);
  char* p = reinterpret_cast<char*>((reinterpret_cast<uintptr_t>(workspace) + 255) & ~uintptr_t(255));
  int64_t a_rows = transA ? K : M, a_cols = transA ? M : K;
  int64_t b_rows = transB ? N : K, b_cols = transB ? K : N;
  void* Ap = p;
  void* Bp = p + tc_prepared_bytes(a_rows, (int)a_cols, prec);
  int rc;
  if ((rc = tc_prepare(A, a_rows, (int)a_cols, lda, prec, Ap, st))) return rc;
  if ((rc = tc_prepare(B, b_rows, (int)b_cols, ldb, prec, Bp, st))) return rc;
  GemmProblem g{};
  g.M = M; g.N = N; g.K = K; g.groups = 1; g.groups_inner = 0;
  StoreEpi epi = make_store_epi(C, ldc, 0, 0);
  return tc_gemm_store(prec, transA != 0, transB == 0, tc_operand(Ap, a_rows, (int)a_cols, prec),
                       tc_operand(Bp, b_rows, (int)b_cols, prec), g, false, epi, st);
}

}
```

### coper_b200/csrc/umma_gemm.cuh

```cuda
#pragma once
#include "umma.cuh"

namespace coper {
namespace umma {

constexpr int PREC_BF16 = COPER_PREC_BF16, PREC_TF32X3 = COPER_PREC_TF32X3, PREC_FP16X3 = COPER_PREC_FP16X3;
constexpr int BLOCK_M = 128;
constexpr int NUM_NON_EPI_THREADS = 128;

template <int PREC_, int BLOCK_N_, int STAGES_, int EPI_WARPS_, bool A_MN_, bool B_MN_, int PROMOTE_KB_ = 0,
          int RES_KB_ = 0>
struct GemmCfg {
  static constexpr int PROMOTE_KB = PROMOTE_KB_;
  static constexpr int RES_KB = RES_KB_;
  static constexpr int PREC = PREC_, BLOCK_N = BLOCK_N_, STAGES = STAGES_, EPI_WARPS = EPI_WARPS_;
  static constexpr bool A_MN = A_MN_, B_MN = B_MN_;
  static constexpr int ELEM = (PREC == PREC_TF32X3) ? 4 : 2;
  static constexpr int CHUNK = 128 / ELEM;
  static constexpr int BLOCK_K = CHUNK;
  static constexpr int UMMA_K = 32 / ELEM;
  static constexpr int TERMS = (PREC == PREC_BF16) ? 1 : 2;
  static constexpr bool SCALED = (PREC == PREC_FP16X3);
  static constexpr int A_BYTES = BLOCK_M * 128;
  static constexpr int B_BYTES = BLOCK_N * 128;
  static constexpr int STAGE_BYTES = RES_KB_ > 0 ? TERMS * A_BYTES : TERMS * (A_BYTES + B_BYTES);
  static constexpr int RES_BYTES = RES_KB_ * TERMS * B_BYTES;
  static constexpr int TMEM_COLS = (2 * BLOCK_N <= 32) ? 32 : (2 * BLOCK_N <= 64) ? 64 : (2 * BLOCK_N <= 128) ? 128
                                   : (2 * BLOCK_N <= 256) ? 256 : 512;
  static constexpr int THREADS = NUM_NON_EPI_THREADS + EPI_WARPS * 32;
  static constexpr size_t SMEM_BYTES = (size_t)STAGES * STAGE_BYTES + RES_BYTES + 1024  + 256 ;

  static constexpr uint32_t FMT = (PREC == PREC_BF16) ? FMT_BF16 : (PREC == PREC_FP16X3) ? FMT_F16 : FMT_TF32;
  static constexpr bool MN_ATOM32 = (PREC == PREC_TF32X3);
  static constexpr uint32_t MN_LAYOUT = MN_ATOM32 ? LAYOUT_SW128_BASE32B : LAYOUT_SW128;
  static constexpr uint32_t MN_SBO = MN_ATOM32 ? 512 : 1024;
  static constexpr uint32_t IDESC = make_idesc(FMT, BLOCK_M, BLOCK_N, A_MN ? 1u : 0u, B_MN ? 1u : 0u);
  static_assert(BLOCK_N % 16 == 0 && BLOCK_N >= 16 && BLOCK_N <= 256, "UMMA N");
  static_assert(2 * BLOCK_N <= 512, "TMEM double buffer");
  static_assert(!A_MN || (BLOCK_M % CHUNK == 0), "MN-major A chunking");
  static_assert(!B_MN || (BLOCK_N % CHUNK == 0), "MN-major B chunking");
};

template <class Cfg>
struct SmemLayout {
  uint8_t* base;
  uint64_t* full;
  uint64_t* empty;
  uint64_t* tfull;
  uint64_t* tempty;
  uint64_t* bfull;
  uint32_t* tmem_ptr;
  uint8_t* res;
  __device__ __forceinline__ explicit SmemLayout(uint8_t* raw) {
    base = reinterpret_cast<uint8_t*>((reinterpret_cast<uintptr_t>(raw) + 1023) & ~uintptr_t(1023));
    res = base + (size_t)Cfg::STAGES * Cfg::STAGE_BYTES;
    uint64_t* bars = reinterpret_cast<uint64_t*>(res + Cfg::RES_BYTES);
    full = bars;
    empty = bars + Cfg::STAGES;
    tfull = bars + 2 * Cfg::STAGES;
    tempty = tfull + 2;
    bfull = tempty + 2;
    tmem_ptr = reinterpret_cast<uint32_t*>(bfull + 1);
  }
  __device__ __forceinline__ uint8_t* res_plane(int kb, int term) const {
    return res + ((size_t)kb * Cfg::TERMS + term) * Cfg::B_BYTES;
  }
  __device__ __forceinline__ uint8_t* a_plane(int stage, int term) const {
    return base + (size_t)stage * Cfg::STAGE_BYTES + term * Cfg::A_BYTES;
  }
  __device__ __forceinline__ uint8_t* b_plane(int stage, int term) const {
    return base + (size_t)stage * Cfg::STAGE_BYTES + Cfg::TERMS * Cfg::A_BYTES + term * Cfg::B_BYTES;
  }
};

template <class Cfg>
__device__ __forceinline__ uint32_t cta_setup(const SmemLayout<Cfg>& sm) {
  int warp = threadIdx.x >> 5;
  if (warp == 1 && (threadIdx.x & 31) == 0) {
    for (int i = 0; i < Cfg::STAGES; ++i) { mbar_init(&sm.full[i], 1); mbar_init(&sm.empty[i], 1); }
    for (int i = 0; i < 2; ++i) { mbar_init(&sm.tfull[i], 1); mbar_init(&sm.tempty[i], Cfg::EPI_WARPS); }
    mbar_init(sm.bfull, 1);
    fence_barrier_init();
  } else if (warp == 2) {
    tmem_alloc(sm.tmem_ptr, Cfg::TMEM_COLS);
    tmem_relinquish();
  }
  tc_fence_before();
  __syncthreads();
  tc_fence_after();
  return *sm.tmem_ptr;
}
template <class Cfg>
__device__ __forceinline__ void cta_teardown(uint32_t tmem_base) {
  tc_fence_before();
  __syncthreads();
  if ((threadIdx.x >> 5) == 2) {
    tc_fence_after();
    tmem_dealloc(tmem_base, Cfg::TMEM_COLS);
  }
}

template <class Cfg>
__device__ __forceinline__ void produce_stage(const SmemLayout<Cfg>& sm, int stage, const CUtensorMap* tA,
                                              const CUtensorMap* tAlo, const CUtensorMap* tB, const CUtensorMap* tBlo,
                                              int a_mn0, int b_mn0, int a_k0, int b_k0, bool leader) {
  uint64_t* bar = &sm.full[stage];
  if (leader) mbar_expect_tx(bar, Cfg::STAGE_BYTES);
#pragma unroll
  for (int t = 0; t < Cfg::TERMS; ++t) {
    const CUtensorMap* ma = t ? tAlo : tA;
    const CUtensorMap* mb = t ? tBlo : tB;
    if (!Cfg::A_MN) {
      if (leader) tma_load_2d(sm.a_plane(stage, t), ma, bar, a_k0, a_mn0);
    } else {
#pragma unroll
      for (int c = 0; c < BLOCK_M / Cfg::CHUNK; ++c)
        if (leader) tma_load_2d(sm.a_plane(stage, t) + c * (Cfg::BLOCK_K * 128), ma, bar, a_mn0 + c * Cfg::CHUNK, a_k0);
    }
    if (Cfg::RES_KB > 0) {
    } else if (!Cfg::B_MN) {
      if (leader) tma_load_2d(sm.b_plane(stage, t), mb, bar, b_k0, b_mn0);
    } else {
#pragma unroll
      for (int c = 0; c < Cfg::BLOCK_N / Cfg::CHUNK; ++c)
        if (leader) tma_load_2d(sm.b_plane(stage, t) + c * (Cfg::BLOCK_K * 128), mb, bar, b_mn0 + c * Cfg::CHUNK, b_k0);
    }
  }
}

template <class Cfg>
__device__ __forceinline__ void issue_stage_rt(const SmemLayout<Cfg>& sm, int stage, uint32_t tmem_d, int kvalid,
                                               bool first, uint32_t idesc, int kb_res, bool leader) {
  const int nk = (kvalid + Cfg::UMMA_K - 1) / Cfg::UMMA_K;
  uint64_t da[2], db[2];
#pragma unroll
  for (int t = 0; t < Cfg::TERMS; ++t) {
    const uint32_t a_addr = smem_u32(sm.a_plane(stage, t));
    const uint32_t b_addr = smem_u32(Cfg::RES_KB > 0 ? sm.res_plane(kb_res, t) : sm.b_plane(stage, t));
    da[t] = Cfg::A_MN ? make_desc(a_addr, Cfg::BLOCK_K * 128, Cfg::MN_SBO, Cfg::MN_LAYOUT) : make_desc_kmajor(a_addr);
    db[t] = Cfg::B_MN ? make_desc(b_addr, Cfg::BLOCK_K * 128, Cfg::MN_SBO, Cfg::MN_LAYOUT) : make_desc_kmajor(b_addr);
  }
  constexpr uint64_t a_step = (Cfg::A_MN ? Cfg::UMMA_K * 128 : 32) >> 4, b_step = (Cfg::B_MN ? Cfg::UMMA_K * 128 : 32) >> 4;
  constexpr int NK_MAX = Cfg::BLOCK_K / Cfg::UMMA_K;
  if (leader) {
#pragma unroll
    for (int k = 0; k < NK_MAX; ++k) {
      if (k < nk) {
        const uint32_t acc = (first && k == 0) ? 0u : 1u;
        if (Cfg::PREC == PREC_BF16) {
          mma_bf16(tmem_d, da[0] + k * a_step, db[0] + k * b_step, idesc, acc);
        } else if (Cfg::PREC == PREC_FP16X3) {
          mma_bf16(tmem_d, da[1] + k * a_step, db[0] + k * b_step, idesc, acc);
          mma_bf16(tmem_d, da[0] + k * a_step, db[1] + k * b_step, idesc, 1u);
          mma_bf16(tmem_d, da[0] + k * a_step, db[0] + k * b_step, idesc, 1u);
        } else {
          mma_tf32(tmem_d, da[1] + k * a_step, db[0] + k * b_step, idesc, acc);
          mma_tf32(tmem_d, da[0] + k * a_step, db[1] + k * b_step, idesc, 1u);
          mma_tf32(tmem_d, da[0] + k * a_step, db[0] + k * b_step, idesc, 1u);
        }
      }
    }
  }
  __syncwarp();
}

struct PipeState {
  int stage = 0;
  uint32_t phase = 0;
  template <int STAGES>
  __device__ __forceinline__ void advance() {
    if (++stage == STAGES) { stage = 0; phase ^= 1; }
  }
};

}
}

namespace coper {
namespace umma {

struct GemmProblem {
  int M, N, K;
  int m_tiles, n_tiles;
  int splits, kb_per_split;
  int groups;
  int groups_inner;
  int a_group_mn, a_group_k;
  int b_group_mn, b_group_k;
  const int* exp_a;
  const int* exp_b;
  float post_scale;
  int n_fastest;
};
struct TileCoord {
  int group, split, m_blk, n_blk, kb0, kb1;
};

struct EpiBase {
  static constexpr bool kAccumulate = false;
  __device__ __forceinline__ void tile_begin(const GemmProblem&, const TileCoord&, int, int) {}
  __device__ __forceinline__ void tile_prefetch(const GemmProblem&, const TileCoord&, int, int) {}
  __device__ __forceinline__ float group_scale(const GemmProblem&, const TileCoord&, int) const { return 1.0f; }
  __device__ __forceinline__ void group_vals(const GemmProblem&, const TileCoord&, int, int, const uint32_t (&)[16],
                                             int) {}
  __device__ __forceinline__ void group_done(const GemmProblem&, const TileCoord&, int, int, int) {}
  __device__ __forceinline__ void tile_done(const GemmProblem&, const TileCoord&, int, int, int) {}
  __device__ __forceinline__ void finish(int, int) {}
};

__device__ __forceinline__ long long gemm_supers(const GemmProblem& p) {
  return (long long)p.m_tiles * p.n_tiles * p.splits * (p.groups_inner ? 1 : p.groups);
}
__device__ __forceinline__ TileCoord gemm_decode(const GemmProblem& p, long long s, int g_inner, int block_k) {
  TileCoord t;
  if (p.n_fastest) {
    t.n_blk = (int)(s % p.n_tiles); s /= p.n_tiles;
    t.m_blk = (int)(s % p.m_tiles); s /= p.m_tiles;
  } else {
    t.m_blk = (int)(s % p.m_tiles); s /= p.m_tiles;
    t.n_blk = (int)(s % p.n_tiles); s /= p.n_tiles;
  }
  t.split = (int)(s % p.splits);  s /= p.splits;
  t.group = p.groups_inner ? g_inner : (int)s;
  int kb_total = (p.K + block_k - 1) / block_k;
  t.kb0 = t.split * p.kb_per_split;
  t.kb1 = min(kb_total, t.kb0 + p.kb_per_split);
  return t;
}

template <class Cfg, class Epi>
__global__ void __launch_bounds__(Cfg::THREADS, 1)
umma_gemm_kernel(const __grid_constant__ CUtensorMap tA, const __grid_constant__ CUtensorMap tAlo,
                 const __grid_constant__ CUtensorMap tB, const __grid_constant__ CUtensorMap tBlo,
                 const GemmProblem p, Epi epi) {
  coper::pdl_trigger();
  extern __shared__ uint8_t smem_raw[];
  SmemLayout<Cfg> sm(smem_raw);
  uint32_t tmem_base = cta_setup<Cfg>(sm);
  coper::pdl_wait();
  const int warp = warp_idx_uniform(), lane = threadIdx.x & 31;
  const long long supers = gemm_supers(p);
  const int g_loop = p.groups_inner ? p.groups : 1;

  if (warp == 0) {
    const bool leader = elect_one();
    if (leader) {
      tma_prefetch_desc(&tA);
      tma_prefetch_desc(&tB);
    }
    PipeState ps;
    int res_nblk = -1;
    for (long long s = blockIdx.x; s < supers; s += gridDim.x) {
      for (int g = 0; g < g_loop; ++g) {
        TileCoord t = gemm_decode(p, s, g, Cfg::BLOCK_K);
        int a_mn0 = t.m_blk * BLOCK_M + t.group * p.a_group_mn;
        int b_mn0 = t.n_blk * Cfg::BLOCK_N + t.group * p.b_group_mn;
        if (Cfg::RES_KB > 0 && t.n_blk != res_nblk) {
          PipeState q = ps;
          for (int i = 0; i < Cfg::STAGES; ++i) {
            mbar_wait(&sm.empty[q.stage], q.phase ^ 1);
            q.template advance<Cfg::STAGES>();
          }
          const int kbn = t.kb1 - t.kb0;
          if (leader) mbar_expect_tx(sm.bfull, (uint32_t)(kbn * Cfg::TERMS * Cfg::B_BYTES));
          for (int kb = t.kb0; kb < t.kb1; ++kb)
#pragma unroll
            for (int tm = 0; tm < Cfg::TERMS; ++tm) {
              if (!Cfg::B_MN) {
                if (leader)
                  tma_load_2d(sm.res_plane(kb - t.kb0, tm), tm ? &tBlo : &tB, sm.bfull, kb * Cfg::BLOCK_K, b_mn0);
              } else {
#pragma unroll
                for (int c = 0; c < Cfg::BLOCK_N / Cfg::CHUNK; ++c)
                  if (leader)
                    tma_load_2d(sm.res_plane(kb - t.kb0, tm) + c * (Cfg::BLOCK_K * 128), tm ? &tBlo : &tB, sm.bfull,
                                b_mn0 + c * Cfg::CHUNK, kb * Cfg::BLOCK_K);
              }
            }
          res_nblk = t.n_blk;
        }
        for (int kb = t.kb0; kb < t.kb1; ++kb) {
          mbar_wait(&sm.empty[ps.stage], ps.phase ^ 1);
          produce_stage<Cfg>(sm, ps.stage, &tA, &tAlo, &tB, &tBlo, a_mn0, b_mn0,
                             kb * Cfg::BLOCK_K + t.group * p.a_group_k, kb * Cfg::BLOCK_K + t.group * p.b_group_k, leader);
          ps.template advance<Cfg::STAGES>();
        }
      }
    }
    __syncwarp();
  } else if (warp == 1) {
    const bool leader = elect_one();
    PipeState ps;
    int as = 0;
    uint32_t aphase = 0;
    int res_nblk = -1;
    uint32_t bphase = 0;
    for (long long s = blockIdx.x; s < supers; s += gridDim.x) {
      for (int g = 0; g < g_loop; ++g) {
        TileCoord t = gemm_decode(p, s, g, Cfg::BLOCK_K);
        if (Cfg::RES_KB > 0 && t.n_blk != res_nblk) {
          mbar_wait(sm.bfull, bphase);
          bphase ^= 1;
          res_nblk = t.n_blk;
        }
        int n_rem = p.N - t.n_blk * Cfg::BLOCK_N;
        int n_eff = min(Cfg::BLOCK_N, (n_rem + 15) & ~15);
        uint32_t idesc = make_idesc(Cfg::FMT, BLOCK_M, (uint32_t)n_eff, Cfg::A_MN ? 1u : 0u, Cfg::B_MN ? 1u : 0u);
        const int chain = Cfg::PROMOTE_KB > 0 ? Cfg::PROMOTE_KB : (t.kb1 - t.kb0);
        for (int kc = t.kb0; kc < t.kb1; kc += chain) {
          int kce = min(t.kb1, kc + chain);
          mbar_wait(&sm.tempty[as], aphase ^ 1);
          tc_fence_after();
          for (int kb = kc; kb < kce; ++kb) {
            mbar_wait(&sm.full[ps.stage], ps.phase);
            tc_fence_after();
            int kvalid = min(Cfg::BLOCK_K, p.K - kb * Cfg::BLOCK_K);
            issue_stage_rt<Cfg>(sm, ps.stage, tmem_base + as * Cfg::BLOCK_N, kvalid, kb == kc, idesc, kb - t.kb0, leader);
            if (leader) mma_commit(&sm.empty[ps.stage]);
            ps.template advance<Cfg::STAGES>();
          }
          if (leader) mma_commit(&sm.tfull[as]);
          __syncwarp();
          as ^= 1;
          if (as == 0) aphase ^= 1;
        }
      }
    }
  } else if (warp >= 4) {
    const int quarter = warp & 3;
    const int group_c = (warp - 4) >> 2;
    constexpr int GROUPS = Cfg::EPI_WARPS / 4;
    constexpr int COLS = Cfg::BLOCK_N / GROUPS;
    constexpr int NCH = COLS / 32;
    static_assert(COLS % 32 == 0, "epilogue column split");
    int as = 0;
    uint32_t aphase = 0;
    const uint32_t lane_base = (uint32_t)(quarter * 32) << 16;
    float acc_scale = 1.0f;
    if (Cfg::SCALED) {
      const int e = (p.exp_a ? __ldg(p.exp_a) : 0) + (p.exp_b ? __ldg(p.exp_b) : 0);
      acc_scale = exp2f((float)-e) * (p.post_scale != 0.f ? p.post_scale : 1.0f);
    }
    for (long long s = blockIdx.x; s < supers; s += gridDim.x) {
      TileCoord t = gemm_decode(p, s, 0, Cfg::BLOCK_K);
      const int row = t.m_blk * BLOCK_M + quarter * 32 + lane;
      const int col0 = t.n_blk * Cfg::BLOCK_N + group_c * COLS;
      epi.tile_begin(p, t, row, col0);
      if (s + gridDim.x < supers) {
        const TileCoord t2 = gemm_decode(p, s + gridDim.x, 0, Cfg::BLOCK_K);
        epi.tile_prefetch(p, t2, t2.m_blk * BLOCK_M + quarter * 32 + lane, t2.n_blk * Cfg::BLOCK_N + group_c * COLS);
      }
      if constexpr (Cfg::PROMOTE_KB == 0 && !Epi::kAccumulate) {
        mbar_wait(&sm.tfull[as], aphase);
        tc_fence_after();
#pragma unroll
        for (int i = 0; i < NCH; ++i) {
          const int col = col0 + i * 32;
          if (col < p.N) {
            uint32_t r[32];
            tmem_ld32(tmem_base + as * Cfg::BLOCK_N + group_c * COLS + i * 32 + lane_base, r);
            tmem_ld_wait();
            if (Cfg::SCALED) {
#pragma unroll
              for (int j = 0; j < 32; ++j) r[j] = __float_as_uint(__uint_as_float(r[j]) * acc_scale);
            }
            epi.chunk(p, t, row, col, r, i);
          }
        }
        tc_fence_before();
        __syncwarp();
        if (lane == 0) mbar_arrive(&sm.tempty[as]);
        as ^= 1;
        if (as == 0) aphase ^= 1;
      } else {
        float accr[NCH][32];
#pragma unroll
        for (int i = 0; i < NCH; ++i)
#pragma unroll
          for (int j = 0; j < 32; ++j) accr[i][j] = 0.f;
        for (int g = 0; g < g_loop; ++g) {
          t = gemm_decode(p, s, g, Cfg::BLOCK_K);
          const float scale = epi.group_scale(p, t, row);
          const int chain = Cfg::PROMOTE_KB > 0 ? Cfg::PROMOTE_KB : (t.kb1 - t.kb0);
          for (int kc = t.kb0; kc < t.kb1; kc += chain) {
            mbar_wait(&sm.tfull[as], aphase);
            tc_fence_after();
#pragma unroll
            for (int i = 0; i < NCH; ++i) {
              if (col0 + i * 32 < p.N) {
#pragma unroll
                for (int h = 0; h < 2; ++h) {
                  uint32_t r[16];
                  tmem_ld16(tmem_base + as * Cfg::BLOCK_N + group_c * COLS + i * 32 + h * 16 + lane_base, r);
                  tmem_ld_wait();
                  if (Cfg::SCALED) {
#pragma unroll
                    for (int j = 0; j < 16; ++j) r[j] = __float_as_uint(__uint_as_float(r[j]) * acc_scale);
                  }
                  epi.group_vals(p, t, row, col0 + i * 32 + h * 16, r, i * 2 + h);
#pragma unroll
                  for (int j = 0; j < 16; ++j) accr[i][h * 16 + j] = fmaf(scale, __uint_as_float(r[j]), accr[i][h * 16 + j]);
                }
              }
            }
            tc_fence_before();
            __syncwarp();
            if (lane == 0) mbar_arrive(&sm.tempty[as]);
            as ^= 1;
            if (as == 0) aphase ^= 1;
          }
          epi.group_done(p, t, row, group_c, GROUPS);
        }
#pragma unroll
        for (int i = 0; i < NCH; ++i) {
          const int col = col0 + i * 32;
          if (col < p.N) {
            uint32_t r[32];
#pragma unroll
            for (int j = 0; j < 32; ++j) r[j] = __float_as_uint(accr[i][j]);
            epi.chunk(p, t, row, col, r, i);
          }
        }
      }
      epi.tile_done(p, t, row, group_c, GROUPS);
    }
    epi.finish(threadIdx.x - NUM_NON_EPI_THREADS, Cfg::EPI_WARPS * 32);
  }
  cta_teardown<Cfg>(tmem_base);
}

struct TcOperand {
  const void* main;
  const void* lo;
  const int* exp;
  uint64_t rows, cols;
  uint64_t pitch;
};

template <class Cfg>
int make_gemm_tmaps(const TcOperand& A, const TcOperand& B, CUtensorMap* tA, CUtensorMap* tAlo, CUtensorMap* tB,
                    CUtensorMap* tBlo) {
  constexpr bool bf16 = Cfg::ELEM == 2;
  int rc;
  uint32_t a_box_rows = Cfg::A_MN ? Cfg::BLOCK_K : BLOCK_M;
  uint32_t b_box_rows = Cfg::B_MN ? Cfg::BLOCK_K : Cfg::BLOCK_N;
  const bool a32 = Cfg::A_MN && Cfg::MN_ATOM32, b32 = Cfg::B_MN && Cfg::MN_ATOM32;
  if ((rc = make_tmap_2d(tA, A.main, Cfg::ELEM, bf16, A.rows, A.cols, A.pitch, Cfg::CHUNK, a_box_rows, a32))) return rc;
  if ((rc = make_tmap_2d(tB, B.main, Cfg::ELEM, bf16, B.rows, B.cols, B.pitch, Cfg::CHUNK, b_box_rows, b32))) return rc;
  *tAlo = *tA;
  *tBlo = *tB;
  if (Cfg::TERMS == 2) {
    if (!A.lo || !B.lo) return COPER_ERR_INVALID_ARG;
    if ((rc = make_tmap_2d(tAlo, A.lo, Cfg::ELEM, bf16, A.rows, A.cols, A.pitch, Cfg::CHUNK, a_box_rows, a32))) return rc;
    if ((rc = make_tmap_2d(tBlo, B.lo, Cfg::ELEM, bf16, B.rows, B.cols, B.pitch, Cfg::CHUNK, b_box_rows, b32))) return rc;
  }
  return COPER_OK;
}

template <class Cfg, class Epi>
int launch_gemm(const TcOperand& A, const TcOperand& B, const GemmProblem& p, const Epi& epi, cudaStream_t st,
                int grid_override = 0) {
  if (p.groups_inner && !Epi::kAccumulate) return COPER_ERR_INVALID_ARG;
  if (Cfg::RES_KB > 0 && (p.splits != 1 || p.groups != 1 || (p.K + Cfg::BLOCK_K - 1) / Cfg::BLOCK_K > Cfg::RES_KB))
    return COPER_ERR_UNSUPPORTED;
  CUtensorMap tA, tAlo, tB, tBlo;
  int rc = make_gemm_tmaps<Cfg>(A, B, &tA, &tAlo, &tB, &tBlo);
  if (rc) return rc;
  int dev = 0;
  if ((rc = check_cuda(cudaGetDevice(&dev)))) return rc;
  static bool attr_done[64] = {};
  if (dev < 0 || dev >= 64) return COPER_ERR_UNSUPPORTED;
  if (!attr_done[dev]) {
    rc = check_cuda(cudaFuncSetAttribute(umma_gemm_kernel<Cfg, Epi>, cudaFuncAttributeMaxDynamicSharedMemorySize,
                                         (int)Cfg::SMEM_BYTES));
    if (rc) return rc;
    attr_done[dev] = true;
  }
  GemmProblem pp = p;
  if (Cfg::SCALED) {
    if (!pp.exp_a) pp.exp_a = A.exp;
    if (!pp.exp_b) pp.exp_b = B.exp;
  }
  const int sms = sm_count();
  long long supers = (long long)p.m_tiles * p.n_tiles * p.splits * (p.groups_inner ? 1 : p.groups);
  int grid = (int)(supers < sms ? supers : sms);
  if (grid_override > 0 && grid_override < grid) grid = grid_override;
  if (grid < 1) return COPER_ERR_INVALID_ARG;
  launch_pdl(umma_gemm_kernel<Cfg, Epi>, grid, Cfg::THREADS, Cfg::SMEM_BYTES, st, tA, tAlo, tB, tBlo, pp, epi);
  return check_launch();
}

template <class Cfg>
inline void plan_gemm(GemmProblem& p, bool allow_split, int target_ctas = 0) {
  if (target_ctas <= 0) target_ctas = sm_count();
  p.m_tiles = (p.M + BLOCK_M - 1) / BLOCK_M;
  p.n_tiles = (p.N + Cfg::BLOCK_N - 1) / Cfg::BLOCK_N;
  int kb_total = (p.K + Cfg::BLOCK_K - 1) / Cfg::BLOCK_K;
  long long base = (long long)p.m_tiles * p.n_tiles * (p.groups_inner ? 1 : p.groups);
  int splits = 1;
  if (allow_split && base < target_ctas) {
    splits = (int)((target_ctas + base - 1) / base);
    if (splits > kb_total) splits = kb_total;
  }
  p.kb_per_split = (kb_total + splits - 1) / splits;
  p.splits = (kb_total + p.kb_per_split - 1) / p.kb_per_split;
}

__device__ __forceinline__ void staged_store_f32(float4* st, const float (&v)[32], float* out0, long long ld,
                                                 int rows_valid, int cols_valid) {
  const int lane = threadIdx.x & 31;
#pragma unroll
  for (int g = 0; g < 8; ++g)
    st[lane * 8 + (g ^ (lane & 7))] = make_float4(v[4 * g], v[4 * g + 1], v[4 * g + 2], v[4 * g + 3]);
  __syncwarp();
  const int g = lane & 7;
#pragma unroll
  for (int k = 0; k < 8; ++k) {
    const int rr = 4 * k + (lane >> 3);
    const float4 x = st[rr * 8 + (g ^ (rr & 7))];
    if (rr < rows_valid && 4 * g < cols_valid) *reinterpret_cast<float4*>(out0 + (long long)rr * ld + 4 * g) = x;
  }
  __syncwarp();
}
constexpr int kStageWarps = 8;
__device__ __forceinline__ float4* stage_tile() {
  __shared__ float4 stage_s[kStageWarps][256];
  return stage_s[((threadIdx.x >> 5) - 4) & (kStageWarps - 1)];
}

struct StoreEpi : EpiBase {
  float* out;
  long long ld, group_stride, split_stride;
  const float* row_scale;
  int row_scale_ld;
  const float* col_bias;
  int extra_col;
  float* extra_out;
  double* sumsq_part;
  double ss_acc;
  __device__ __forceinline__ void chunk(const GemmProblem& p, const TileCoord& t, int row, int col,
                                        const uint32_t (&r)[32], int) {
    const int lane = threadIdx.x & 31;
    const int n_out = extra_col >= 0 ? min(p.N, extra_col) : p.N;
    if (sumsq_part && row < p.M) {
      float ss = 0.f;
#pragma unroll
      for (int j = 0; j < 32; ++j) {
        const float v = __uint_as_float(r[j]);
        ss = (col + j < n_out) ? fmaf(v, v, ss) : ss;
      }
      ss_acc += (double)ss;
    }
    float* base = out + t.group * group_stride + t.split * split_stride;
    float* o0 = base + (long long)(row - lane) * ld + col;
    const bool vec = !col_bias && !row_scale && extra_col < 0 && ((ld & 3) == 0) && ((n_out & 3) == 0) &&
                     ((reinterpret_cast<uintptr_t>(o0) & 15) == 0);
    if (vec) {
      float v[32];
#pragma unroll
      for (int j = 0; j < 32; ++j) v[j] = __uint_as_float(r[j]);
      staged_store_f32(stage_tile(), v, o0, ld, p.M - (row - lane), n_out - col);
      return;
    }
    if (row >= p.M) return;
    float sc = row_scale ? __ldg(row_scale + (long long)row * row_scale_ld + t.group) : 1.0f;
    float* o = base + (long long)row * ld + col;
    {
#pragma unroll
      for (int j = 0; j < 32; ++j) {
        int cj = col + j;
        if (cj < n_out) o[j] = __uint_as_float(r[j]) * sc + (col_bias ? __ldg(col_bias + cj) : 0.f);
        else if (cj == extra_col && cj < p.N) extra_out[row] = __uint_as_float(r[j]) * sc;
      }
    }
  }
  __device__ __forceinline__ void finish(int epi_thread, int epi_threads) {
    if (!sumsq_part) return;
    const double t = warp_sum_d(ss_acc);
    if ((epi_thread & 31) == 0) sumsq_part[(long long)blockIdx.x * (epi_threads >> 5) + (epi_thread >> 5)] = t;
  }
};

inline StoreEpi make_store_epi(float* out, long long ld, long long group_stride, long long split_stride) {
  StoreEpi e;
  e.out = out; e.ld = ld; e.group_stride = group_stride; e.split_stride = split_stride;
  e.row_scale = nullptr; e.row_scale_ld = 0; e.col_bias = nullptr; e.extra_col = -1; e.extra_out = nullptr;
  e.sumsq_part = nullptr; e.ss_acc = 0.0;
  return e;
}

}
}
```

### include/coper.h

```cpp
#ifndef COPER_H_
#define COPER_H_

#include <stdint.h>
#include <stddef.h>

#ifdef __cplusplus
extern "C" {
#endif

typedef void* coper_stream_t;

typedef enum {
  COPER_OK = 0,
  COPER_ERR_INVALID_ARG = -1,
  COPER_ERR_CUDA = -2,
  COPER_ERR_UNSUPPORTED = -3,
  COPER_ERR_WORKSPACE = -4
} coper_status;

enum { COPER_PREC_FP32 = 0, COPER_PREC_BF16 = 1, COPER_PREC_TF32X3 = 2, COPER_PREC_FP16X3 = 3 };

int coper_version(void);
const char* coper_status_string(int status);
int coper_last_cuda_error(void);
long long coper_launch_count(void);
int coper_set_pdl(int on);
int coper_device_is_sm100(void);

int coper_gather_rows(const float* table, int64_t row_lo, int64_t row_hi, int width,
                      const int64_t* idx, int n_idx, float* out, coper_stream_t stream);
int coper_gather_rows2(const float* table_a, int64_t lo_a, int64_t hi_a, int width_a, const int64_t* idx_a, int n_a,
                       float* out_a, const float* table_b, int64_t lo_b, int64_t hi_b, int width_b,
                       const int64_t* idx_b, int n_b, float* out_b, float* step_state, uint64_t* seed_dev, float lr,
                       float beta1, float beta2, coper_stream_t stream);

int coper_conv_fwd(const float* x0, int B, int H, int W, const float* wc, const float* bc, int KH, int KW,
                   int C, int per_query, float* z, coper_stream_t stream);
int coper_conv_bwd_slabs(int B, int H, int W, int KH, int KW, int C, int per_query);
int coper_conv_bwd(const float* dz, const float* x0, int B, int H, int W, const float* wc, int KH, int KW,
                   int C, int per_query, float* dx0, float* dwc_part, float* dbc_part, coper_stream_t stream);
int coper_conv_bwd_bn(const float* dout, const float* z, const float* x0, int B, int H, int W, const float* wc, int KH,
                      int KW, int C, int per_query, const float* a, const float* b, const float* mean,
                      const float* invstd, const float* c1, const float* c2, int relu, float keep_post,
                      const uint64_t* seed_dev, uint64_t salt_post, float* dx0, float* dwc_part, float* dbc_part,
                      float* dz_scratch, coper_stream_t stream);

int coper_colstats_chunks(int64_t R);
int coper_colstats(const float* x, int64_t R, int C, float* partials, coper_stream_t stream);
int coper_bn_finalize(const float* partials, int nchunk, int64_t R, int C, const float* gamma, const float* beta,
                      float* moving_mean, float* moving_var, float momentum, float eps, int use_batch_stats,
                      int update_moving, int bessel, float* a, float* b, float* mean, float* invstd,
                      coper_stream_t stream);
int coper_bn_stats_finalize(const float* x, int64_t R, int C, float* partials, unsigned int* sync_word,
                            const float* gamma, const float* beta, float* moving_mean, float* moving_var,
                            float momentum, float eps, int update_moving, int bessel, float* a, float* b, float* mean,
                            float* invstd, coper_stream_t stream);
int coper_bn_act_fwd(const float* x, int64_t R, int C, const float* a, const float* b, int relu,
                     float keep_post, const uint64_t* seed_dev, uint64_t salt_post, float* out, coper_stream_t stream);
int coper_bn_act_fwd_moving(const float* x, int64_t R, int C, const float* gamma, const float* beta,
                            const float* moving_mean, const float* moving_var, float eps, int relu, float* out,
                            coper_stream_t stream);
int coper_bn_act_bwd_stats(const float* dout, const float* x, int64_t R, int C, const float* a, const float* b,
                           const float* mean, const float* invstd, int relu, float keep_post,
                           const uint64_t* seed_dev, uint64_t salt_post, float* partials, coper_stream_t stream);
int coper_bn_act_bwd_finalize(const float* partials, int nchunk, int64_t R, int C, int use_batch_stats,
                              float* dgamma, float* dbeta, float* c1, float* c2, coper_stream_t stream);
int coper_bn_act_bwd_stats_finalize(const float* dout, const float* x, int64_t R, int C, const float* a, const float* b,
                                    const float* mean, const float* invstd, int relu, float keep_post,
                                    const uint64_t* seed_dev, uint64_t salt_post, float* partials,
                                    unsigned int* sync_word, int use_batch_stats, float* dgamma, float* dbeta, float* c1,
                                    float* c2, coper_stream_t stream);
int coper_bn_act_bwd_apply(const float* dout, const float* x, int64_t R, int C, const float* a, const float* b,
                           const float* mean, const float* invstd, const float* c1, const float* c2, int relu,
                           float keep_post, const uint64_t* seed_dev, uint64_t salt_post, float keep_pre,
                           uint64_t salt_pre, float* dx, coper_stream_t stream);
int coper_dropout_mask(int64_t n, float keep, const uint64_t* seed_dev, uint64_t salt, float* mask,
                       coper_stream_t stream);
int coper_dropout_apply(float* x, int64_t n, float keep, const uint64_t* seed_dev, uint64_t salt,
                        coper_stream_t stream);

size_t coper_cpg_fc_fwd_workspace_bytes(int B, int dc, int F, int d, int prec);
int coper_cpg_fc_fwd(const float* c, const float* f, const float* P, const void* P_prepared, const float* cb,
                     const float* Pb, int B, int dc, int F, int d, int dcb, float keep_out, const uint64_t* seed_dev,
                     uint64_t salt_out, float* y, void* workspace, size_t workspace_bytes, int prec,
                     coper_stream_t stream);
#define COPER_CPG_BWD_REUSE_FWD 1
#define COPER_CPG_BWD_INPUT_GRADS_ONLY 2
#define COPER_CPG_BWD_WEIGHT_GRADS_ONLY 4
#define COPER_CPG_BWD_DCB_ACCUMULATE 8
size_t coper_cpg_fc_bwd_workspace_bytes(int B, int dc, int F, int d, int prec);
int coper_cpg_fc_bwd(const float* c, const float* f, const float* P, const void* P_prepared, const float* cb,
                     const float* Pb, const float* dy, int B, int dc, int F, int d, int dcb, float* dP, float* dPb, float* df,
                     float* dc_out, float* dcb_out, void* workspace, size_t workspace_bytes, int prec,
                     int flags, coper_stream_t stream);

int coper_sgemm(int transA, int transB, int M, int N, int K, const float* A, int lda, const float* B, int ldb,
                float* C, int ldc, int accumulate, coper_stream_t stream);

size_t coper_score1n_workspace_bytes(int B, int64_t Ns, int d, int prec);
int coper_score1n_fwd(const float* q, const float* E, const float* bias, int B, int64_t Ns, int d, float* scores,
                      int64_t ld_scores, void* workspace, size_t workspace_bytes, int prec, coper_stream_t stream);

size_t coper_prepared_bytes(int64_t rows, int cols, int prec);
int coper_prepare_operand(const float* src, int64_t rows, int cols, int64_t ld_src, int prec, void* dst,
                          coper_stream_t stream);
int coper_score1n_fwd_prepared(const void* q_prep, const void* E_prep, const float* bias, int B, int64_t Ns, int d,
                               float* scores, int64_t ld_scores, int prec, coper_stream_t stream);

size_t coper_tc_gemm_workspace_bytes(int M, int N, int K, int prec);
int coper_tc_gemm(int transA, int transB, int M, int N, int K, const float* A, int lda, const float* B, int ldb,
                  float* C, int ldc, int prec, void* workspace, size_t workspace_bytes, coper_stream_t stream);

size_t coper_score1n_bce_workspace_bytes(int B, int64_t Ns, int d, int prec);
size_t coper_score1n_bce_G_bytes(int B, int64_t Ns, int prec);
int coper_score1n_bce_fwd_bwd(const float* q, const float* E, const void* E_prepared, const float* bias,
                              const uint32_t* label_bits,
                              int B, int64_t Ns, int d, float pos_target, float neg_target, float inv_count,
                              double* loss_sum, void* G, int64_t ldG, float* dq, float* dE, float* dbias,
                              void* workspace, size_t workspace_bytes, int prec, coper_stream_t stream);

int coper_score1n_bce_fwd_bwd_norm(const float* q, const float* E, const void* E_prepared, const float* bias,
                                   const uint32_t* label_bits, int B, int64_t Ns, int d, float pos_target,
                                   float neg_target, float inv_count, double* loss_sum, void* G, int64_t ldG, float* dq,
                                   float* dE, float* dbias, double* dE_sumsq, void* workspace, size_t workspace_bytes,
                                   int prec, coper_stream_t stream);

int coper_score1n_bce_dE(const void* G, int B, int64_t Ns, int d, float inv_count, float* dE, double* dE_sumsq,
                         float* dbias, void* workspace, size_t workspace_bytes, int prec, coper_stream_t stream);

size_t coper_score_sampled_workspace_bytes(int B, int L);

int coper_sample_labels(const int32_t* rowptr, const int32_t* col, int B, int64_t N, int L, int n_pos_needed,
                        const uint64_t* seed_dev, uint64_t salt, int32_t* lookup, float* labels, coper_stream_t stream);
int coper_score_sampled_bce_fwd_bwd(const float* q, const float* E, const float* bias, const int32_t* lookup,
                                    const float* labels, int B, int L, int64_t N, int d, float one_minus_eps,
                                    float inv_num_ent, float inv_count, double* loss_sum, float* scores, float* g,
                                    float* dq, float* dE_sum, float* dE_sq, float* dbias_sum, float* dbias_sq,
                                    void* workspace, size_t workspace_bytes, coper_stream_t stream);

size_t coper_score_sampled_sharded_workspace_bytes(int B, int L);
int coper_score_sampled_bce_fwd_bwd_sharded(const float* q, const float* E, const float* bias, const int32_t* lookup,
                                            const float* labels, int B, int L, int64_t N, int d, float one_minus_eps,
                                            float inv_num_ent, float inv_count, double* loss_sum, float* scores,
                                            float* g, float* dq, float* dE_sum, float* dE_sq, float* dbias_sum,
                                            float* dbias_sq, int64_t row_lo, int64_t row_hi, void* workspace,
                                            size_t workspace_bytes, coper_stream_t stream);

int coper_score_candidates(const float* q, const float* E, const float* bias, const int32_t* cand, int B, int C, int d,
                           int64_t row_lo, int64_t row_hi, float* scores, coper_stream_t stream);
int coper_candidate_rank(const float* q, const float* E, const float* bias, const int32_t* cand, const int32_t* e2,
                         int B, int C, int d, int64_t row_lo, int64_t row_hi, const float* gold,
                         const uint32_t* filter_bits, int entity_major, int32_t* n_greater, int32_t* n_equal,
                         coper_stream_t stream);

int coper_csr_to_bits(const int32_t* rowptr, const int32_t* col, int B, int64_t ent_lo, int64_t ent_hi,
                      uint32_t* bits, coper_stream_t stream);
int coper_dense_to_bits(const float* dense, int B, int64_t N, uint32_t* bits, coper_stream_t stream);
int coper_csr_to_bits_t(const int32_t* rowptr, const int32_t* col, int B, int64_t ent_lo, int64_t ent_hi,
                        uint32_t* bits_t, coper_stream_t stream);
int coper_dense_to_bits_t(const float* dense, int B, int64_t N, int64_t ld_dense, uint32_t* bits_t,
                          coper_stream_t stream);
int coper_bits_t_set(const int64_t* ent, int B, int64_t ent_lo, int64_t ent_hi, uint32_t* bits_t,
                     coper_stream_t stream);

int coper_gold_scores(const float* scores, int64_t ld, int B, int64_t Ns, const int64_t* e2, int64_t ent_lo,
                      float* gold, coper_stream_t stream);
int coper_filtered_rank(const float* scores, int64_t ld, int B, int64_t Ns, const int64_t* e2, int64_t ent_lo,
                        const float* gold, const uint32_t* filter_bits, int32_t* n_greater, int32_t* n_equal,
                        coper_stream_t stream);

size_t coper_score1n_rank_workspace_bytes(int B, int d, int prec);
int coper_score1n_gold_prepared(const void* q_prep, const void* E_prep, const float* bias, int B, int64_t Ns, int d,
                                const int64_t* e2, int64_t ent_lo, float* gold, void* workspace,
                                size_t workspace_bytes, int prec, coper_stream_t stream);
int coper_score1n_rank_prepared(const void* q_prep, const void* E_prep, const float* bias, int B, int64_t Ns, int d,
                                const float* gold, const uint32_t* filter_bits_t, int32_t* n_greater,
                                int32_t* n_equal, int prec, coper_stream_t stream);

#define COPER_TOPK_MAX 128
size_t coper_score1n_topk_workspace_bytes(int B, int64_t Ns, int d, int k, int prec);
int coper_score1n_topk_prepared(const void* q_prep, const void* E_prep, const float* bias, int B, int64_t Ns, int d,
                                const uint32_t* filter_bits_t, int64_t ent_lo, int k, float* out_scores,
                                int64_t* out_ids, void* workspace, size_t workspace_bytes, int prec,
                                coper_stream_t stream);
size_t coper_topk_scores_workspace_bytes(int B, int64_t Ns, int k);
int coper_topk_scores(const float* scores, int64_t ld, int B, int64_t Ns, const uint32_t* filter_bits, int64_t ent_lo,
                      int k, float* out_scores, int64_t* out_ids, void* workspace, size_t workspace_bytes,
                      coper_stream_t stream);
int coper_topk_merge(const float* in_scores, const int64_t* in_ids, int n_lists, int B, int k, float* out_scores,
                     int64_t* out_ids, coper_stream_t stream);

size_t coper_segscatter_workspace_bytes(int M);
int coper_segscatter_add_sq(const int64_t* idx, int M, const float* src, int width, float* dst, float* dst_sq,
                            int64_t row_lo, int64_t row_hi, coper_stream_t stream);
int coper_segscatter_add_norm(const int64_t* idx, int M, const float* src, int width, float* dst, float* dst_sq,
                              int64_t row_lo, int64_t row_hi, double* norm_delta, coper_stream_t stream);
int coper_segscatter_add_pair(const int64_t* idx_a, int M_a, const float* src_a, int width_a, float* dst_a,
                              float* dst_sq_a, int64_t lo_a, int64_t hi_a, double* norm_delta_a, const int64_t* idx_b,
                              int M_b, const float* src_b, int width_b, float* dst_b, float* dst_sq_b, int64_t lo_b,
                              int64_t hi_b, coper_stream_t stream);
int coper_segscatter_add(const int64_t* idx, int M, const float* src, int width, float* dst, int64_t row_lo,
                         int64_t row_hi, void* workspace, size_t workspace_bytes, coper_stream_t stream);

#define COPER_SUMSQ_BLOCKS 256
int coper_reduce_partials(const float* in, int S, int64_t n, float scale, int accumulate, float* out,
                          coper_stream_t stream);
int coper_reduce_partials2(const float* in_a, int64_t n_a, float* out_a, const float* in_b, int64_t n_b, float* out_b,
                           int S, float scale, int accumulate, coper_stream_t stream);
int coper_sumsq(const float* x, int64_t n, int slot, double* partials, coper_stream_t stream);
int coper_clip_scale(const double* partials, int n_slots, float clip_norm, float* out2, coper_stream_t stream);

int coper_step_state_advance(float* step_state, uint64_t* seed_dev, float lr, float beta1, float beta2,
                             coper_stream_t stream);
int coper_amsgrad_step(float* theta, const float* grad, float* m, float* v, float* vhat, int64_t n,
                       const float* step_state, float beta1, float beta2, float eps, const float* clip_scale,
                       int bug_compat, coper_stream_t stream);

#define COPER_MT_CHUNK 16384
enum { COPER_GRAD_DENSE = 0, COPER_GRAD_INDEXED_SLICES = 1, COPER_GRAD_NORM_EXTERNAL = 2 };
typedef struct {
  float* theta;
  const float* grad;
  float* m;
  float* v;
  float* vhat;
  void* prepared;
  const float* grad_sq;
  int64_t n;
  int32_t prepared_prec;
  int32_t mode;
} coper_param_desc;
int coper_sumsq_combine(const double* parts, int n_parts, const double* deltas, int n_deltas, double* out,
                        coper_stream_t stream);
int coper_mt_sumsq(const coper_param_desc* descs, int n_tensors, const int32_t* chunks, int n_chunks,
                   const int32_t* chunk_offsets, double* chunk_partials, double* tensor_sumsq, coper_stream_t stream);
int coper_clip_scale_n(const double* sums, int n, float clip_norm, float* out2, coper_stream_t stream);
int coper_mt_sumsq_clip(const coper_param_desc* descs, int n_tensors, const int32_t* chunks, int n_chunks,
                        const int32_t* chunk_offsets, double* chunk_partials, double* tensor_sumsq, int ext_tensor,
                        const double* ext_parts, int n_ext_parts, const double* ext_deltas, int n_ext_deltas,
                        float clip_norm, float* clip_out, coper_stream_t stream);
int coper_mt_amsgrad(const coper_param_desc* descs, const int32_t* chunks, int n_chunks, const float* step_state,
                     float beta1, float beta2, float eps, const float* clip_scale, int bug_compat,
                     coper_stream_t stream);

#ifdef __cplusplus
}
#endif
#endif
```

Before: 999,200.

## Add thread-block-cluster TMA multicast path for fp16x3 UMMA GEMMs

Adds an optional cluster launch (2 or 4 CTAs) for fp16x3 GEMM configs whose shared memory permits only one CTA per SM. Within a cluster the B operand tile is split across CTAs and loaded once with TMA multicast, and stage release is signalled through a multicast tcgen05 commit. A planner queries cluster occupancy and uses a cluster only when it does not add scheduling rounds. This is meant to cut L2/global traffic for the shared operand in the dE, dq and CPG GEMMs, at the cost of cross-CTA synchronisation and possibly fewer resident CTAs.

```diff
diff --git a/coper_b200/_lib.py b/coper_b200/_lib.py
--- a/coper_b200/_lib.py
+++ b/coper_b200/_lib.py
@@ -98,6 +98,7 @@
     "coper_mt_sumsq_clip": (i32, [vp, i32, vp, i32, vp, vp, vp, i32, vp, i32, vp, i32, f32, vp, vp]),
     "coper_mt_amsgrad": (i32, [vp, vp, i32, vp, f32, f32, f32, vp, i32, vp]),
     "coper_amsgrad_step": (i32, [vp, vp, vp, vp, vp, i64, vp, f32, f32, f32, vp, i32, vp]),
+    "coper_gemm_cluster": (i32, [i32, i32, i64, i32, i32, i32]),
 }
 SUMSQ_BLOCKS = 256
 TOPK_MAX = 128
diff --git a/coper_b200/csrc/common.cuh b/coper_b200/csrc/common.cuh
--- a/coper_b200/csrc/common.cuh
+++ b/coper_b200/csrc/common.cuh
@@ -40,18 +40,27 @@
 }
 bool pdl_enabled();
 template <typename... KArgs, typename... Args>
-inline void launch_pdl(void (*kernel)(KArgs...), dim3 grid, dim3 block, size_t smem, cudaStream_t st, Args&&... args) {
+inline void launch_pdl_cluster(void (*kernel)(KArgs...), dim3 grid, dim3 block, size_t smem, int cluster,
+                               cudaStream_t st, Args&&... args) {
   cudaLaunchConfig_t cfg = {};
   cfg.gridDim = grid;
   cfg.blockDim = block;
   cfg.dynamicSmemBytes = smem;
   cfg.stream = st;
-  cudaLaunchAttribute attr[1];
+  cudaLaunchAttribute attr[2];
   attr[0].id = cudaLaunchAttributeProgrammaticStreamSerialization;
   attr[0].val.programmaticStreamSerializationAllowed = pdl_enabled() ? 1 : 0;
+  attr[1].id = cudaLaunchAttributeClusterDimension;
+  attr[1].val.clusterDim.x = (unsigned)cluster;
+  attr[1].val.clusterDim.y = 1;
+  attr[1].val.clusterDim.z = 1;
   cfg.attrs = attr;
-  cfg.numAttrs = 1;
+  cfg.numAttrs = cluster > 1 ? 2 : 1;
   cudaLaunchKernelEx(&cfg, kernel, static_cast<KArgs>(args)...);
+}
+template <typename... KArgs, typename... Args>
+inline void launch_pdl(void (*kernel)(KArgs...), dim3 grid, dim3 block, size_t smem, cudaStream_t st, Args&&... args) {
+  launch_pdl_cluster(kernel, grid, block, smem, 1, st, static_cast<Args&&>(args)...);
 }
 
 __host__ __device__ __forceinline__ uint32_t hash32(uint64_t seed, uint64_t idx) {
diff --git a/coper_b200/csrc/umma.cuh b/coper_b200/csrc/umma.cuh
--- a/coper_b200/csrc/umma.cuh
+++ b/coper_b200/csrc/umma.cuh
@@ -45,6 +45,23 @@
       "cp.async.bulk.tensor.2d.shared::cluster.global.mbarrier::complete_tx::bytes [%0], [%1, {%3, %4}], [%2];"
       ::"r"(smem_u32(dst_smem)), "l"(reinterpret_cast<uint64_t>(tmap)), "r"(smem_u32(bar)), "r"(c0), "r"(c1)
       : "memory");
+}
+__device__ __forceinline__ void tma_load_2d_mc(void* dst_smem, const CUtensorMap* tmap, uint64_t* bar, int c0, int c1,
+                                               uint16_t cta_mask) {
+  asm volatile(
+      "cp.async.bulk.tensor.2d.shared::cluster.global.mbarrier::complete_tx::bytes.multicast::cluster"
+      " [%0], [%1, {%3, %4}], [%2], %5;"
+      ::"r"(smem_u32(dst_smem)), "l"(reinterpret_cast<uint64_t>(tmap)), "r"(smem_u32(bar)), "r"(c0), "r"(c1),
+        "h"(cta_mask)
+      : "memory");
+}
+__device__ __forceinline__ uint32_t cluster_ctarank() {
+  uint32_t r;
+  asm volatile("mov.u32 %0, %%cluster_ctarank;" : "=r"(r));
+  return r;
+}
+__device__ __forceinline__ void cluster_sync() {
+  asm volatile("barrier.cluster.arrive.release;\n\tbarrier.cluster.wait.acquire;" ::: "memory");
 }
 __device__ __forceinline__ void tma_store_2d(const CUtensorMap* tmap, const void* src_smem, int c0, int c1) {
   asm volatile("cp.async.bulk.tensor.2d.global.shared::cta.bulk_group [%0, {%2, %3}], [%1];"
@@ -113,6 +130,11 @@
   asm volatile("tcgen05.commit.cta_group::1.mbarrier::arrive::one.shared::cluster.b64 [%0];" ::"r"(smem_u32(bar))
                : "memory");
 }
+__device__ __forceinline__ void mma_commit_mc(uint64_t* bar, uint16_t cta_mask) {
+  asm volatile("tcgen05.commit.cta_group::1.mbarrier::arrive::one.shared::cluster.multicast::cluster.b64 [%0], %1;"
+               ::"r"(smem_u32(bar)), "h"(cta_mask)
+               : "memory");
+}
 
 __device__ __forceinline__ void tmem_ld32(uint32_t taddr, uint32_t (&r)[32]) {
   asm volatile(
diff --git a/coper_b200/csrc/umma_cpg.cu b/coper_b200/csrc/umma_cpg.cu
--- a/coper_b200/csrc/umma_cpg.cu
+++ b/coper_b200/csrc/umma_cpg.cu
@@ -10,7 +10,8 @@
 TcOperand tc_operand(const void* prep, int64_t rows, int cols, int prec);
 void* tc_fp16x3_trailer(const void* prep, int64_t rows, int cols);
 int tc_gemm_store(int prec, bool a_mn, bool b_mn, const TcOperand& A, const TcOperand& B, const GemmProblem& p,
-                  bool split, const StoreEpi& epi, cudaStream_t st);
+                  bool split, const StoreEpi& epi, cudaStream_t st, bool cluster);
+int tc_store_cluster(int prec, bool a_mn, bool b_mn, GemmProblem p, bool split, bool cluster);
 
 struct CpgFwdEpi : EpiBase {
   static constexpr bool kAccumulate = true;
@@ -51,9 +52,9 @@
   GemmProblem p{};
   p.M = B; p.N = d; p.K = F; p.groups = dc; p.groups_inner = 1;
   p.a_group_mn = 0; p.a_group_k = 0; p.b_group_mn = 0; p.b_group_k = F;
-  if (prec == COPER_PREC_BF16) plan_gemm<CpgFwdCfg<PREC_BF16>>(p, true);
-  else if (prec == COPER_PREC_FP16X3) plan_gemm<CpgFwdCfg<PREC_FP16X3>>(p, true);
-  else plan_gemm<CpgFwdCfg<PREC_TF32X3>>(p, true);
+  if (prec == COPER_PREC_BF16) plan_gemm<CpgFwdCfg<PREC_BF16>>(p, true, 0, true);
+  else if (prec == COPER_PREC_FP16X3) plan_gemm<CpgFwdCfg<PREC_FP16X3>>(p, true, 0, true);
+  else plan_gemm<CpgFwdCfg<PREC_TF32X3>>(p, true, 0, true);
   L.p = p;
   size_t o = 0;
   L.off_f = o; o = align_up(o + tc_prepared_bytes(B, F, prec), 256);
@@ -236,6 +237,29 @@
     *reinterpret_cast<uint4*>(hi) = *reinterpret_cast<uint4*>(h);
     *reinterpret_cast<uint4*>(lo) = *reinterpret_cast<uint4*>(l);
   }
+}
+
+static GemmProblem cpg_t_problem(int B, int dc, int F, int d, int prec) {
+  GemmProblem p{};
+  p.M = B; p.N = F; p.K = d; p.groups = dc; p.groups_inner = 1;
+  p.a_group_mn = 0; p.a_group_k = 0; p.b_group_mn = F; p.b_group_k = 0;
+  if (prec == COPER_PREC_BF16) plan_gemm<CpgBwdTCfg<PREC_BF16>>(p, false, 0, true);
+  else if (prec == COPER_PREC_FP16X3) plan_gemm<CpgBwdTCfg<PREC_FP16X3>>(p, false, 0, true);
+  else plan_gemm<CpgBwdTCfg<PREC_TF32X3>>(p, false, 0, true);
+  return p;
+}
+static GemmProblem cpg_dp_problem(int B, int dc, int F, int d) {
+  GemmProblem p{};
+  p.M = F; p.N = d; p.K = B; p.groups = dc; p.groups_inner = 0;
+  p.a_group_mn = 0; p.a_group_k = 0; p.b_group_mn = 0; p.b_group_k = B;
+  return p;
+}
+int umma_cpg_gemm_cluster(int kind, int B, int dc, int F, int d, int prec) {
+  GemmProblem p{};
+  if (kind == COPER_GEMM_CPG_FWD) p = cpg_fwd_plan(B, dc, F, d, prec).p;
+  else if (kind == COPER_GEMM_CPG_T) p = cpg_t_problem(B, dc, F, d, prec);
+  else return tc_store_cluster(prec, true, true, cpg_dp_problem(B, dc, F, d), false, true);
+  return p.cluster > 1 ? p.cluster : 1;
 }
 
 struct CpgBwdPlan {
@@ -330,33 +354,21 @@
       launch_pdl(prepare_scaled_kernel, grid, 256, 0, st, dy, c, B, d, dc, ldp, prec, dycp, trailer);
       if ((rc = check_launch())) return rc;
     }
-    GemmProblem p{};
-    p.M = B; p.N = F; p.K = d; p.groups = dc; p.groups_inner = 1;
-    p.a_group_mn = 0; p.a_group_k = 0; p.b_group_mn = F; p.b_group_k = 0;
+    GemmProblem p = cpg_t_problem(B, dc, F, d, prec);
     CpgBwdTEpi epi;
     epi.c = c; epi.f = f; epi.dc = dc; epi.df = df; epi.dc_part = dc_part; epi.fsum = 0.f;
     TcOperand A = tc_operand(dyp, B, d, prec), Bo = tc_operand(Pp, (int64_t)dc * F, d, prec);
-    if (prec == COPER_PREC_BF16) {
-      plan_gemm<CpgBwdTCfg<PREC_BF16>>(p, false);
-      rc = launch_gemm<CpgBwdTCfg<PREC_BF16>, CpgBwdTEpi>(A, Bo, p, epi, st);
-    } else if (prec == COPER_PREC_FP16X3) {
-      plan_gemm<CpgBwdTCfg<PREC_FP16X3>>(p, false);
-      rc = launch_gemm<CpgBwdTCfg<PREC_FP16X3>, CpgBwdTEpi>(A, Bo, p, epi, st);
-    } else {
-      plan_gemm<CpgBwdTCfg<PREC_TF32X3>>(p, false);
-      rc = launch_gemm<CpgBwdTCfg<PREC_TF32X3>, CpgBwdTEpi>(A, Bo, p, epi, st);
-    }
+    if (prec == COPER_PREC_BF16) rc = launch_gemm<CpgBwdTCfg<PREC_BF16>, CpgBwdTEpi>(A, Bo, p, epi, st);
+    else if (prec == COPER_PREC_FP16X3) rc = launch_gemm<CpgBwdTCfg<PREC_FP16X3>, CpgBwdTEpi>(A, Bo, p, epi, st);
+    else rc = launch_gemm<CpgBwdTCfg<PREC_TF32X3>, CpgBwdTEpi>(A, Bo, p, epi, st);
     if (rc) return rc;
     if ((rc = coper_reduce_partials(dc_part, L.dc_slabs, (int64_t)B * dc, 1.0f, 0, dc_out, (coper_stream_t)st)))
       return rc;
   }
   if (weights) {
-    GemmProblem p{};
-    p.M = F; p.N = d; p.K = B; p.groups = dc; p.groups_inner = 0;
-    p.a_group_mn = 0; p.a_group_k = 0; p.b_group_mn = 0; p.b_group_k = B;
     StoreEpi epi = make_store_epi(dP, d, (long long)F * d, 0);
-    rc = tc_gemm_store(prec, true, true, tc_operand(fp, B, F, prec), tc_operand(dycp, (int64_t)dc * B, d, prec), p,
-                       false, epi, st);
+    rc = tc_gemm_store(prec, true, true, tc_operand(fp, B, F, prec), tc_operand(dycp, (int64_t)dc * B, d, prec),
+                       cpg_dp_problem(B, dc, F, d), false, epi, st, true);
   }
   return rc;
 }
diff --git a/coper_b200/csrc/umma_entity.cu b/coper_b200/csrc/umma_entity.cu
--- a/coper_b200/csrc/umma_entity.cu
+++ b/coper_b200/csrc/umma_entity.cu
@@ -11,7 +11,8 @@
 TcOperand tc_operand(const void* prep, int64_t rows, int cols, int prec);
 void* tc_fp16x3_trailer(const void* prep, int64_t rows, int cols);
 int tc_gemm_store(int prec, bool a_mn, bool b_mn, const TcOperand& A, const TcOperand& B, const GemmProblem& p,
-                  bool split, const StoreEpi& epi, cudaStream_t st);
+                  bool split, const StoreEpi& epi, cudaStream_t st, bool cluster);
+int tc_store_cluster(int prec, bool a_mn, bool b_mn, GemmProblem p, bool split, bool cluster);
 int tc_plan_splits(int prec, GemmProblem p, bool split);
 bool umma_fused_ok(int B, int64_t Ns, int d, int prec);
 void umma_fused_plan(int B, int64_t Ns, int* QB, int* R);
@@ -606,6 +607,21 @@
   ENT_DISPATCH(topk_impl, E, Q, bias, B, Ns, d, filtT, ent_lo, k, out_s, out_id, ws, st);
 }
 
+static GemmProblem dq_problem(int B, int64_t Ns, int d) {
+  GemmProblem p{};
+  p.M = B; p.N = d; p.K = (int)Ns; p.groups = 1; p.groups_inner = 0;
+  return p;
+}
+static GemmProblem dE_problem(int B, int64_t Ns, int d) {
+  GemmProblem p{};
+  p.M = (int)Ns; p.N = d; p.K = B; p.groups = 1; p.groups_inner = 0;
+  return p;
+}
+int umma_bce_gemm_cluster(int kind, int B, int64_t Ns, int d, int prec) {
+  const bool entity_major = prec != COPER_PREC_TF32X3;
+  if (kind == COPER_GEMM_DQ) return tc_store_cluster(prec, entity_major, true, dq_problem(B, Ns, d), true, true);
+  return tc_store_cluster(prec, !entity_major, true, dE_problem(B, Ns, d), false, true);
+}
 static int dE_gemm(int prec, bool a_mn, const TcOperand& Go, const TcOperand& Qo, const GemmProblem& p, StoreEpi epi,
                    double* dE_sumsq, double* ss_part, cudaStream_t st) {
   int rc;
@@ -614,7 +630,7 @@
     if ((rc = check_cuda(cudaMemsetAsync(ss_part, 0, (size_t)n_part * sizeof(double), st)))) return rc;
     epi.sumsq_part = ss_part;
   }
-  if ((rc = tc_gemm_store(prec, a_mn, true, Go, Qo, p, false, epi, st))) return rc;
+  if ((rc = tc_gemm_store(prec, a_mn, true, Go, Qo, p, false, epi, st, true))) return rc;
   if (dE_sumsq) {
     launch_pdl(sum_doubles_kernel, 1, 256, 0, st, ss_part, n_part, dE_sumsq);
     rc = check_launch();
@@ -712,8 +728,7 @@
     if (rc) return rc;
   }
   TcOperand Qo = tc_operand(w + L.off_q, B, d, prec), Go = g_operand(G, B, Ns, prec);
-  GemmProblem p{};
-  p.M = (int)Ns; p.N = d; p.K = B; p.groups = 1; p.groups_inner = 0;
+  GemmProblem p = dE_problem(B, Ns, d);
   p.post_scale = prec == COPER_PREC_FP16X3 ? inv_count * (1.0f / 1024.0f) : 0.f;
   StoreEpi epi = make_store_epi(dE, d, 0, 0);
   return dE_gemm(prec, prec == COPER_PREC_TF32X3, Go, Qo, p, epi, dE_sumsq, reinterpret_cast<double*>(w + L.off_ss), st);
@@ -773,11 +788,10 @@
   if ((rc = run_bce())) return rc;
   TcOperand Go = g_operand(G, B, Ns, prec);
   {
-    GemmProblem p{};
-    p.M = B; p.N = d; p.K = (int)Ns; p.groups = 1; p.groups_inner = 0;
+    GemmProblem p = dq_problem(B, Ns, d);
     p.post_scale = g_post;
     StoreEpi epi = make_store_epi(dq_part, d, 0, (long long)B * d);
-    if ((rc = tc_gemm_store(prec, entity_major, true, Go, Eo, p, true, epi, st))) return rc;
+    if ((rc = tc_gemm_store(prec, entity_major, true, Go, Eo, p, true, epi, st, true))) return rc;
     if ((rc = reduce_partials_and_sum(dq_part, L.splits, (int64_t)B * d, 1.0f, 0, dq, loss_part, grid * kBceEpiWarps,
                                       loss_sum, st)))
       return rc;
diff --git a/coper_b200/csrc/umma_gemm.cu b/coper_b200/csrc/umma_gemm.cu
--- a/coper_b200/csrc/umma_gemm.cu
+++ b/coper_b200/csrc/umma_gemm.cu
@@ -7,19 +7,63 @@
 int tc_prepare(const float* src, int64_t rows, int cols, int64_t ld_src, int prec, void* dst, cudaStream_t st);
 int64_t tc_prepared_ld(int cols, int prec);
 void* tc_fp16x3_trailer(const void* prep, int64_t rows, int cols);
+int umma_bce_gemm_cluster(int kind, int B, int64_t Ns, int d, int prec);
+int umma_cpg_gemm_cluster(int kind, int B, int dc, int F, int d, int prec);
 
 template <int PREC, bool A_MN, bool B_MN>
 using StoreCfg = GemmCfg<PREC, 256, (PREC == PREC_BF16 ? 4 : 2), (PREC == PREC_BF16 ? 4 : 8), A_MN, B_MN,
                          (PREC == PREC_BF16 ? 0 : PREC == PREC_FP16X3 ? 2 : 4)>;
 
+template <int PREC, bool A_MN, bool B_MN>
+static int plan_launch(const TcOperand* A, const TcOperand* B, GemmProblem& p, bool split, bool cluster,
+                       const StoreEpi* epi, cudaStream_t st) {
+  plan_gemm<StoreCfg<PREC, A_MN, B_MN>>(p, split, 0, cluster);
+  return A ? launch_gemm<StoreCfg<PREC, A_MN, B_MN>>(*A, *B, p, *epi, st) : COPER_OK;
+}
 template <int PREC>
-static int dispatch_layout(bool a_mn, bool b_mn, const TcOperand& A, const TcOperand& B, GemmProblem p, bool split,
-                           const StoreEpi& epi, cudaStream_t st) {
-  if (!a_mn && !b_mn) { plan_gemm<StoreCfg<PREC, false, false>>(p, split); return launch_gemm<StoreCfg<PREC, false, false>>(A, B, p, epi, st); }
-  if (!a_mn && b_mn)  { plan_gemm<StoreCfg<PREC, false, true>>(p, split);  return launch_gemm<StoreCfg<PREC, false, true>>(A, B, p, epi, st); }
-  if (a_mn && !b_mn)  { plan_gemm<StoreCfg<PREC, true, false>>(p, split);  return launch_gemm<StoreCfg<PREC, true, false>>(A, B, p, epi, st); }
-  plan_gemm<StoreCfg<PREC, true, true>>(p, split);
-  return launch_gemm<StoreCfg<PREC, true, true>>(A, B, p, epi, st);
+static int dispatch_layout(bool a_mn, bool b_mn, const TcOperand* A, const TcOperand* B, GemmProblem& p, bool split,
+                           bool cluster, const StoreEpi* epi, cudaStream_t st) {
+  if (!a_mn && !b_mn) return plan_launch<PREC, false, false>(A, B, p, split, cluster, epi, st);
+  if (!a_mn && b_mn) return plan_launch<PREC, false, true>(A, B, p, split, cluster, epi, st);
+  if (a_mn && !b_mn) return plan_launch<PREC, true, false>(A, B, p, split, cluster, epi, st);
+  return plan_launch<PREC, true, true>(A, B, p, split, cluster, epi, st);
+}
+static int dispatch_prec(int prec, bool a_mn, bool b_mn, const TcOperand* A, const TcOperand* B, GemmProblem& p,
+                         bool split, bool cluster, const StoreEpi* epi, cudaStream_t st) {
+  if (prec == COPER_PREC_BF16) return dispatch_layout<PREC_BF16>(a_mn, b_mn, A, B, p, split, cluster, epi, st);
+  if (prec == COPER_PREC_TF32X3) return dispatch_layout<PREC_TF32X3>(a_mn, b_mn, A, B, p, split, cluster, epi, st);
+  if (prec == COPER_PREC_FP16X3) return dispatch_layout<PREC_FP16X3>(a_mn, b_mn, A, B, p, split, cluster, epi, st);
+  return COPER_ERR_UNSUPPORTED;
+}
+
+__global__ void cluster_probe_kernel() { pdl_enter(); }
+int umma::cluster_capacity(int cluster) {
+  static int cached[64][5] = {};
+  int dev = 0;
+  if (cluster < 1 || cluster > 4 || cudaGetDevice(&dev) != cudaSuccess || dev < 0 || dev >= 64) return 0;
+  int& c = cached[dev][cluster];
+  if (c == 0) {
+    constexpr int kSmem = 160 * 1024;
+    int n = 0;
+    cudaLaunchConfig_t cfg = {};
+    cfg.gridDim = dim3(cluster * 64);
+    cfg.blockDim = dim3(128);
+    cfg.dynamicSmemBytes = kSmem;
+    cudaLaunchAttribute a[1];
+    a[0].id = cudaLaunchAttributeClusterDimension;
+    a[0].val.clusterDim.x = (unsigned)cluster;
+    a[0].val.clusterDim.y = 1;
+    a[0].val.clusterDim.z = 1;
+    cfg.attrs = a;
+    cfg.numAttrs = 1;
+    if (cudaFuncSetAttribute(cluster_probe_kernel, cudaFuncAttributeMaxDynamicSharedMemorySize, kSmem) != cudaSuccess ||
+        cudaOccupancyMaxActiveClusters(&n, cluster_probe_kernel, &cfg) != cudaSuccess) {
+      cudaGetLastError();
+      n = 0;
+    }
+    c = n > 0 ? n : -1;
+  }
+  return c > 0 ? c : 0;
 }
 
 using ResBCfg = GemmCfg<PREC_BF16, 128, 4, 8, false, true, 0, 8>;
@@ -33,11 +77,13 @@
 }
 
 int tc_gemm_store(int prec, bool a_mn, bool b_mn, const TcOperand& A, const TcOperand& B, const GemmProblem& p,
-                  bool split, const StoreEpi& epi, cudaStream_t st) {
-  if (prec == COPER_PREC_BF16) return dispatch_layout<PREC_BF16>(a_mn, b_mn, A, B, p, split, epi, st);
-  if (prec == COPER_PREC_TF32X3) return dispatch_layout<PREC_TF32X3>(a_mn, b_mn, A, B, p, split, epi, st);
-  if (prec == COPER_PREC_FP16X3) return dispatch_layout<PREC_FP16X3>(a_mn, b_mn, A, B, p, split, epi, st);
-  return COPER_ERR_UNSUPPORTED;
+                  bool split, const StoreEpi& epi, cudaStream_t st, bool cluster) {
+  GemmProblem q = p;
+  return dispatch_prec(prec, a_mn, b_mn, &A, &B, q, split, cluster, &epi, st);
+}
+int tc_store_cluster(int prec, bool a_mn, bool b_mn, GemmProblem p, bool split, bool cluster) {
+  int rc = dispatch_prec(prec, a_mn, b_mn, nullptr, nullptr, p, split, cluster, nullptr, nullptr);
+  return rc ? rc : (p.cluster > 1 ? p.cluster : 1);
 }
 int tc_plan_splits(int prec, GemmProblem p, bool split) {
   if (prec == COPER_PREC_BF16) plan_gemm<StoreCfg<PREC_BF16, false, false>>(p, split);
@@ -89,7 +135,20 @@
   g.M = M; g.N = N; g.K = K; g.groups = 1; g.groups_inner = 0;
   StoreEpi epi = make_store_epi(C, ldc, 0, 0);
   return tc_gemm_store(prec, transA != 0, transB == 0, tc_operand(Ap, a_rows, (int)a_cols, prec),
-                       tc_operand(Bp, b_rows, (int)b_cols, prec), g, false, epi, st);
+                       tc_operand(Bp, b_rows, (int)b_cols, prec), g, false, epi, st, false);
+}
+
+int coper_gemm_cluster(int kind, int B, int64_t n, int d, int dc, int prec) {
+  COPER_CHECK_ARG(B > 0 && n > 0 && n < 0x7fffffff && d > 0 && dc > 0);
+  if (prec != COPER_PREC_BF16 && prec != COPER_PREC_TF32X3 && prec != COPER_PREC_FP16X3) return COPER_ERR_UNSUPPORTED;
+  switch (kind) {
+    case COPER_GEMM_DQ:
+    case COPER_GEMM_DE: return umma_bce_gemm_cluster(kind, B, n, d, prec);
+    case COPER_GEMM_CPG_FWD:
+    case COPER_GEMM_CPG_T:
+    case COPER_GEMM_CPG_DP: return umma_cpg_gemm_cluster(kind, B, dc, (int)n, d, prec);
+  }
+  return COPER_ERR_INVALID_ARG;
 }
 
 }
diff --git a/coper_b200/csrc/umma_gemm.cuh b/coper_b200/csrc/umma_gemm.cuh
--- a/coper_b200/csrc/umma_gemm.cuh
+++ b/coper_b200/csrc/umma_gemm.cuh
@@ -74,10 +74,10 @@
 };
 
 template <class Cfg>
-__device__ __forceinline__ uint32_t cta_setup(const SmemLayout<Cfg>& sm) {
+__device__ __forceinline__ uint32_t cta_setup(const SmemLayout<Cfg>& sm, int cluster) {
   int warp = threadIdx.x >> 5;
   if (warp == 1 && (threadIdx.x & 31) == 0) {
-    for (int i = 0; i < Cfg::STAGES; ++i) { mbar_init(&sm.full[i], 1); mbar_init(&sm.empty[i], 1); }
+    for (int i = 0; i < Cfg::STAGES; ++i) { mbar_init(&sm.full[i], 1); mbar_init(&sm.empty[i], cluster); }
     for (int i = 0; i < 2; ++i) { mbar_init(&sm.tfull[i], 1); mbar_init(&sm.tempty[i], Cfg::EPI_WARPS); }
     mbar_init(sm.bfull, 1);
     fence_barrier_init();
@@ -87,13 +87,15 @@
   }
   tc_fence_before();
   __syncthreads();
+  if (cluster > 1) cluster_sync();
   tc_fence_after();
   return *sm.tmem_ptr;
 }
 template <class Cfg>
-__device__ __forceinline__ void cta_teardown(uint32_t tmem_base) {
+__device__ __forceinline__ void cta_teardown(uint32_t tmem_base, int cluster) {
   tc_fence_before();
   __syncthreads();
+  if (cluster > 1) cluster_sync();
   if ((threadIdx.x >> 5) == 2) {
     tc_fence_after();
     tmem_dealloc(tmem_base, Cfg::TMEM_COLS);
@@ -103,9 +105,36 @@
 template <class Cfg>
 __device__ __forceinline__ void produce_stage(const SmemLayout<Cfg>& sm, int stage, const CUtensorMap* tA,
                                               const CUtensorMap* tAlo, const CUtensorMap* tB, const CUtensorMap* tBlo,
-                                              int a_mn0, int b_mn0, int a_k0, int b_k0, bool leader) {
+                                              int a_mn0, int b_mn0, int a_k0, int b_k0, bool leader, int cluster,
+                                              int rank) {
   uint64_t* bar = &sm.full[stage];
   if (leader) mbar_expect_tx(bar, Cfg::STAGE_BYTES);
+  if (cluster > 1) {
+    const uint16_t mask = (uint16_t)((1u << cluster) - 1u);
+    constexpr int NBM = Cfg::BLOCK_N / Cfg::CHUNK;
+    const int nb = Cfg::B_MN ? NBM : cluster;
+    const int rows = Cfg::BLOCK_N / cluster;
+#pragma unroll
+    for (int t = 0; t < Cfg::TERMS; ++t) {
+      const CUtensorMap* ma = t ? tAlo : tA;
+      const CUtensorMap* mb = t ? tBlo : tB;
+      if (!Cfg::A_MN) {
+        if (leader) tma_load_2d(sm.a_plane(stage, t), ma, bar, a_k0, a_mn0);
+      } else {
+#pragma unroll
+        for (int c = 0; c < BLOCK_M / Cfg::CHUNK; ++c)
+          if (leader) tma_load_2d(sm.a_plane(stage, t) + c * (Cfg::BLOCK_K * 128), ma, bar, a_mn0 + c * Cfg::CHUNK, a_k0);
+      }
+      for (int i = 0; i < nb; ++i) {
+        if ((t * nb + i) % cluster != rank || !leader) continue;
+        if (Cfg::B_MN)
+          tma_load_2d_mc(sm.b_plane(stage, t) + i * (Cfg::BLOCK_K * 128), mb, bar, b_mn0 + i * Cfg::CHUNK, b_k0, mask);
+        else
+          tma_load_2d_mc(sm.b_plane(stage, t) + i * rows * 128, mb, bar, b_k0, b_mn0 + i * rows, mask);
+      }
+    }
+    return;
+  }
 #pragma unroll
   for (int t = 0; t < Cfg::TERMS; ++t) {
     const CUtensorMap* ma = t ? tAlo : tA;
@@ -191,6 +220,7 @@
   const int* exp_b;
   float post_scale;
   int n_fastest;
+  int cluster;
 };
 struct TileCoord {
   int group, split, m_blk, n_blk, kb0, kb1;
@@ -208,16 +238,21 @@
   __device__ __forceinline__ void finish(int, int) {}
 };
 
-__device__ __forceinline__ long long gemm_supers(const GemmProblem& p) {
-  return (long long)p.m_tiles * p.n_tiles * p.splits * (p.groups_inner ? 1 : p.groups);
-}
-__device__ __forceinline__ TileCoord gemm_decode(const GemmProblem& p, long long s, int g_inner, int block_k) {
+__host__ __device__ __forceinline__ int gemm_m_slots(const GemmProblem& p, int cluster) {
+  return cluster > 1 ? (p.m_tiles + cluster - 1) / cluster * cluster : p.m_tiles;
+}
+__host__ __device__ __forceinline__ long long gemm_supers(const GemmProblem& p, int cluster = 1) {
+  return (long long)gemm_m_slots(p, cluster) * p.n_tiles * p.splits * (p.groups_inner ? 1 : p.groups);
+}
+__device__ __forceinline__ TileCoord gemm_decode(const GemmProblem& p, long long s, int g_inner, int block_k,
+                                                 int cluster = 1) {
   TileCoord t;
   if (p.n_fastest) {
     t.n_blk = (int)(s % p.n_tiles); s /= p.n_tiles;
     t.m_blk = (int)(s % p.m_tiles); s /= p.m_tiles;
   } else {
-    t.m_blk = (int)(s % p.m_tiles); s /= p.m_tiles;
+    const int ms = gemm_m_slots(p, cluster);
+    t.m_blk = (int)(s % ms); s /= ms;
     t.n_blk = (int)(s % p.n_tiles); s /= p.n_tiles;
   }
   t.split = (int)(s % p.splits);  s /= p.splits;
@@ -228,7 +263,7 @@
   return t;
 }
 
-template <class Cfg, class Epi>
+template <class Cfg, class Epi, bool MC = false>
 __global__ void __launch_bounds__(Cfg::THREADS, 1)
 umma_gemm_kernel(const __grid_constant__ CUtensorMap tA, const __grid_constant__ CUtensorMap tAlo,
                  const __grid_constant__ CUtensorMap tB, const __grid_constant__ CUtensorMap tBlo,
@@ -236,10 +271,11 @@
   coper::pdl_trigger();
   extern __shared__ uint8_t smem_raw[];
   SmemLayout<Cfg> sm(smem_raw);
-  uint32_t tmem_base = cta_setup<Cfg>(sm);
+  const int cluster = MC ? p.cluster : 1;
+  uint32_t tmem_base = cta_setup<Cfg>(sm, cluster);
   coper::pdl_wait();
   const int warp = warp_idx_uniform(), lane = threadIdx.x & 31;
-  const long long supers = gemm_supers(p);
+  const long long supers = gemm_supers(p, cluster);
   const int g_loop = p.groups_inner ? p.groups : 1;
 
   if (warp == 0) {
@@ -248,11 +284,12 @@
       tma_prefetch_desc(&tA);
       tma_prefetch_desc(&tB);
     }
+    const int rank = cluster > 1 ? (int)cluster_ctarank() : 0;
     PipeState ps;
     int res_nblk = -1;
     for (long long s = blockIdx.x; s < supers; s += gridDim.x) {
       for (int g = 0; g < g_loop; ++g) {
-        TileCoord t = gemm_decode(p, s, g, Cfg::BLOCK_K);
+        TileCoord t = gemm_decode(p, s, g, Cfg::BLOCK_K, cluster);
         int a_mn0 = t.m_blk * BLOCK_M + t.group * p.a_group_mn;
         int b_mn0 = t.n_blk * Cfg::BLOCK_N + t.group * p.b_group_mn;
         if (Cfg::RES_KB > 0 && t.n_blk != res_nblk) {
@@ -282,14 +319,22 @@
         for (int kb = t.kb0; kb < t.kb1; ++kb) {
           mbar_wait(&sm.empty[ps.stage], ps.phase ^ 1);
           produce_stage<Cfg>(sm, ps.stage, &tA, &tAlo, &tB, &tBlo, a_mn0, b_mn0,
-                             kb * Cfg::BLOCK_K + t.group * p.a_group_k, kb * Cfg::BLOCK_K + t.group * p.b_group_k, leader);
+                             kb * Cfg::BLOCK_K + t.group * p.a_group_k, kb * Cfg::BLOCK_K + t.group * p.b_group_k, leader,
+                             cluster, rank);
           ps.template advance<Cfg::STAGES>();
         }
+      }
+    }
+    if (cluster > 1) {
+      for (int i = 0; i < Cfg::STAGES; ++i) {
+        mbar_wait(&sm.empty[ps.stage], ps.phase ^ 1);
+        ps.template advance<Cfg::STAGES>();
       }
     }
     __syncwarp();
   } else if (warp == 1) {
     const bool leader = elect_one();
+    const uint16_t mask = (uint16_t)((1u << cluster) - 1u);
     PipeState ps;
     int as = 0;
     uint32_t aphase = 0;
@@ -297,7 +342,7 @@
     uint32_t bphase = 0;
     for (long long s = blockIdx.x; s < supers; s += gridDim.x) {
       for (int g = 0; g < g_loop; ++g) {
-        TileCoord t = gemm_decode(p, s, g, Cfg::BLOCK_K);
+        TileCoord t = gemm_decode(p, s, g, Cfg::BLOCK_K, cluster);
         if (Cfg::RES_KB > 0 && t.n_blk != res_nblk) {
           mbar_wait(sm.bfull, bphase);
           bphase ^= 1;
@@ -316,7 +361,10 @@
             tc_fence_after();
             int kvalid = min(Cfg::BLOCK_K, p.K - kb * Cfg::BLOCK_K);
             issue_stage_rt<Cfg>(sm, ps.stage, tmem_base + as * Cfg::BLOCK_N, kvalid, kb == kc, idesc, kb - t.kb0, leader);
-            if (leader) mma_commit(&sm.empty[ps.stage]);
+            if (leader) {
+              if (cluster > 1) mma_commit_mc(&sm.empty[ps.stage], mask);
+              else mma_commit(&sm.empty[ps.stage]);
+            }
             ps.template advance<Cfg::STAGES>();
           }
           if (leader) mma_commit(&sm.tfull[as]);
@@ -342,12 +390,12 @@
       acc_scale = exp2f((float)-e) * (p.post_scale != 0.f ? p.post_scale : 1.0f);
     }
     for (long long s = blockIdx.x; s < supers; s += gridDim.x) {
-      TileCoord t = gemm_decode(p, s, 0, Cfg::BLOCK_K);
+      TileCoord t = gemm_decode(p, s, 0, Cfg::BLOCK_K, cluster);
       const int row = t.m_blk * BLOCK_M + quarter * 32 + lane;
       const int col0 = t.n_blk * Cfg::BLOCK_N + group_c * COLS;
       epi.tile_begin(p, t, row, col0);
       if (s + gridDim.x < supers) {
-        const TileCoord t2 = gemm_decode(p, s + gridDim.x, 0, Cfg::BLOCK_K);
+        const TileCoord t2 = gemm_decode(p, s + gridDim.x, 0, Cfg::BLOCK_K, cluster);
         epi.tile_prefetch(p, t2, t2.m_blk * BLOCK_M + quarter * 32 + lane, t2.n_blk * Cfg::BLOCK_N + group_c * COLS);
       }
       if constexpr (Cfg::PROMOTE_KB == 0 && !Epi::kAccumulate) {
@@ -379,7 +427,7 @@
 #pragma unroll
           for (int j = 0; j < 32; ++j) accr[i][j] = 0.f;
         for (int g = 0; g < g_loop; ++g) {
-          t = gemm_decode(p, s, g, Cfg::BLOCK_K);
+          t = gemm_decode(p, s, g, Cfg::BLOCK_K, cluster);
           const float scale = epi.group_scale(p, t, row);
           const int chain = Cfg::PROMOTE_KB > 0 ? Cfg::PROMOTE_KB : (t.kb1 - t.kb0);
           for (int kc = t.kb0; kc < t.kb1; kc += chain) {
@@ -426,7 +474,7 @@
     }
     epi.finish(threadIdx.x - NUM_NON_EPI_THREADS, Cfg::EPI_WARPS * 32);
   }
-  cta_teardown<Cfg>(tmem_base);
+  cta_teardown<Cfg>(tmem_base, cluster);
 }
 
 struct TcOperand {
@@ -439,11 +487,11 @@
 
 template <class Cfg>
 int make_gemm_tmaps(const TcOperand& A, const TcOperand& B, CUtensorMap* tA, CUtensorMap* tAlo, CUtensorMap* tB,
-                    CUtensorMap* tBlo) {
+                    CUtensorMap* tBlo, int cluster = 1) {
   constexpr bool bf16 = Cfg::ELEM == 2;
   int rc;
   uint32_t a_box_rows = Cfg::A_MN ? Cfg::BLOCK_K : BLOCK_M;
-  uint32_t b_box_rows = Cfg::B_MN ? Cfg::BLOCK_K : Cfg::BLOCK_N;
+  uint32_t b_box_rows = Cfg::B_MN ? Cfg::BLOCK_K : Cfg::BLOCK_N / cluster;
   const bool a32 = Cfg::A_MN && Cfg::MN_ATOM32, b32 = Cfg::B_MN && Cfg::MN_ATOM32;
   if ((rc = make_tmap_2d(tA, A.main, Cfg::ELEM, bf16, A.rows, A.cols, A.pitch, Cfg::CHUNK, a_box_rows, a32))) return rc;
   if ((rc = make_tmap_2d(tB, B.main, Cfg::ELEM, bf16, B.rows, B.cols, B.pitch, Cfg::CHUNK, b_box_rows, b32))) return rc;
@@ -457,41 +505,82 @@
   return COPER_OK;
 }
 
+int cluster_capacity(int cluster);
+template <class Cfg>
+constexpr bool kClusterCfg = Cfg::PREC == PREC_FP16X3 && Cfg::RES_KB == 0 && 2 * Cfg::SMEM_BYTES > 228 * 1024;
+template <class Cfg>
+inline bool cluster_supported(const GemmProblem& p, int cluster) {
+  return kClusterCfg<Cfg> && (cluster == 2 || cluster == 4) && !p.n_fastest && Cfg::BLOCK_N % (8 * cluster) == 0 &&
+         (!Cfg::B_MN || Cfg::TERMS * (Cfg::BLOCK_N / Cfg::CHUNK) >= cluster);
+}
+template <class Cfg>
+inline int plan_cluster(const GemmProblem& p) {
+  if (!kClusterCfg<Cfg>) return 1;
+  const long long per_m = (long long)p.n_tiles * p.splits * (p.groups_inner ? 1 : p.groups);
+  const int sms = sm_count();
+  const long long rounds = ((long long)p.m_tiles * per_m + sms - 1) / sms;
+  for (int c = 4; c >= 2; c >>= 1) {
+    if (p.m_tiles < c || !cluster_supported<Cfg>(p, c)) continue;
+    const long long slots = (long long)cluster_capacity(c) * c;
+    const long long supers = (long long)((p.m_tiles + c - 1) / c * c) * per_m;
+    if (slots > 0 && (supers + slots - 1) / slots <= rounds) return c;
+  }
+  return 1;
+}
+
 template <class Cfg, class Epi>
 int launch_gemm(const TcOperand& A, const TcOperand& B, const GemmProblem& p, const Epi& epi, cudaStream_t st,
                 int grid_override = 0) {
   if (p.groups_inner && !Epi::kAccumulate) return COPER_ERR_INVALID_ARG;
   if (Cfg::RES_KB > 0 && (p.splits != 1 || p.groups != 1 || (p.K + Cfg::BLOCK_K - 1) / Cfg::BLOCK_K > Cfg::RES_KB))
     return COPER_ERR_UNSUPPORTED;
+  const int cluster = p.cluster > 1 ? p.cluster : 1;
+  if (cluster > 1 && !cluster_supported<Cfg>(p, cluster)) return COPER_ERR_UNSUPPORTED;
   CUtensorMap tA, tAlo, tB, tBlo;
-  int rc = make_gemm_tmaps<Cfg>(A, B, &tA, &tAlo, &tB, &tBlo);
+  int rc = make_gemm_tmaps<Cfg>(A, B, &tA, &tAlo, &tB, &tBlo, cluster);
   if (rc) return rc;
   int dev = 0;
   if ((rc = check_cuda(cudaGetDevice(&dev)))) return rc;
-  static bool attr_done[64] = {};
+  static bool attr_done[64][2] = {};
   if (dev < 0 || dev >= 64) return COPER_ERR_UNSUPPORTED;
-  if (!attr_done[dev]) {
+  if (!attr_done[dev][0]) {
     rc = check_cuda(cudaFuncSetAttribute(umma_gemm_kernel<Cfg, Epi>, cudaFuncAttributeMaxDynamicSharedMemorySize,
                                          (int)Cfg::SMEM_BYTES));
     if (rc) return rc;
-    attr_done[dev] = true;
+    attr_done[dev][0] = true;
+  }
+  if constexpr (kClusterCfg<Cfg>) {
+    if (cluster > 1 && !attr_done[dev][1]) {
+      rc = check_cuda(cudaFuncSetAttribute(umma_gemm_kernel<Cfg, Epi, true>,
+                                           cudaFuncAttributeMaxDynamicSharedMemorySize, (int)Cfg::SMEM_BYTES));
+      if (rc) return rc;
+      attr_done[dev][1] = true;
+    }
   }
   GemmProblem pp = p;
   if (Cfg::SCALED) {
     if (!pp.exp_a) pp.exp_a = A.exp;
     if (!pp.exp_b) pp.exp_b = B.exp;
   }
-  const int sms = sm_count();
-  long long supers = (long long)p.m_tiles * p.n_tiles * p.splits * (p.groups_inner ? 1 : p.groups);
-  int grid = (int)(supers < sms ? supers : sms);
+  const int slots = cluster > 1 ? cluster_capacity(cluster) * cluster : sm_count();
+  long long supers = gemm_supers(p, cluster);
+  int grid = (int)(supers < slots ? supers : slots);
   if (grid_override > 0 && grid_override < grid) grid = grid_override;
+  grid = grid / cluster * cluster;
   if (grid < 1) return COPER_ERR_INVALID_ARG;
+  if constexpr (kClusterCfg<Cfg>) {
+    if (cluster > 1) {
+      launch_pdl_cluster(umma_gemm_kernel<Cfg, Epi, true>, grid, Cfg::THREADS, Cfg::SMEM_BYTES, cluster, st, tA, tAlo,
+                         tB, tBlo, pp, epi);
+      return check_launch();
+    }
+  }
   launch_pdl(umma_gemm_kernel<Cfg, Epi>, grid, Cfg::THREADS, Cfg::SMEM_BYTES, st, tA, tAlo, tB, tBlo, pp, epi);
   return check_launch();
 }
 
 template <class Cfg>
-inline void plan_gemm(GemmProblem& p, bool allow_split, int target_ctas = 0) {
+inline void plan_gemm(GemmProblem& p, bool allow_split, int target_ctas = 0, bool allow_cluster = false) {
   if (target_ctas <= 0) target_ctas = sm_count();
   p.m_tiles = (p.M + BLOCK_M - 1) / BLOCK_M;
   p.n_tiles = (p.N + Cfg::BLOCK_N - 1) / Cfg::BLOCK_N;
@@ -504,6 +593,7 @@
   }
   p.kb_per_split = (kb_total + splits - 1) / splits;
   p.splits = (kb_total + p.kb_per_split - 1) / p.kb_per_split;
+  p.cluster = allow_cluster ? plan_cluster<Cfg>(p) : 1;
 }
 
 __device__ __forceinline__ void staged_store_f32(float4* st, const float (&v)[32], float* out0, long long ld,
diff --git a/include/coper.h b/include/coper.h
--- a/include/coper.h
+++ b/include/coper.h
@@ -111,6 +111,9 @@
 int coper_tc_gemm(int transA, int transB, int M, int N, int K, const float* A, int lda, const float* B, int ldb,
                   float* C, int ldc, int prec, void* workspace, size_t workspace_bytes, coper_stream_t stream);
 
+enum { COPER_GEMM_DQ = 0, COPER_GEMM_DE = 1, COPER_GEMM_CPG_FWD = 2, COPER_GEMM_CPG_T = 3, COPER_GEMM_CPG_DP = 4 };
+int coper_gemm_cluster(int kind, int B, int64_t n, int d, int dc, int prec);
+
 size_t coper_score1n_bce_workspace_bytes(int B, int64_t Ns, int d, int prec);
 size_t coper_score1n_bce_G_bytes(int B, int64_t Ns, int prec);
 int coper_score1n_bce_fwd_bwd(const float* q, const float* E, const void* E_prepared, const float* bias,
```

New measurement: 1.026 million, median of 6. +2.7%, better.
